# Z-Zheng/ever

Measured on AMD Instinct MI355X. Metric: 512x512 tiles/sec fwd+bwd, FarSeg-R50, higher is better.
Workload: dtype f32; 1 GPU; FarSeg ResNet-50 FPN (FarSegHead defaults, BCE+dice), 3-band 512x512, batch 16/GPU, fwd+bwd+SGD step, inputs resident in HBM; global_batch=16, parallelism=single

## Files before the change

ever_amd/_C.py:

```python
import ctypes as C
import os

_LIB_PATH = os.path.join(os.path.dirname(os.path.abspath(__file__)), 'lib', 'libever_hip.so')
_LIB_PATH = os.environ.get('EVK_LIB', _LIB_PATH)

c_void_p, c_int, c_i32, c_i64, c_u32, c_f32, c_size_t = (
    C.c_void_p, C.c_int, C.c_int32, C.c_int64, C.c_uint32, C.c_float, C.c_size_t)


class ConvDesc(C.Structure):
    _fields_ = [(n, c_i32) for n in (
        'N', 'H', 'W', 'Cin', 'Ho', 'Wo', 'Cout', 'kh', 'kw',
        'stride_h', 'stride_w', 'pad_h', 'pad_w', 'dil_h', 'dil_w')]


class SplitJob(C.Structure):
    _fields_ = [('w', c_void_p), ('out', c_void_p), ('kind', c_i32), ('arg', c_i32 * 13)]


P = c_void_p
_DP = C.POINTER(ConvDesc)
_JP = C.POINTER(SplitJob)

SIGNATURES = {
    'evk_last_error': (C.c_char_p, []),
    'evk_abi_version': (c_int, []),
    'evk_build_arch': (C.c_char_p, []),
    'evk_conv2d_fwd': (c_int, [_DP, P, P, P, P, c_u32, P]),
    'evk_conv2d_dgrad': (c_int, [_DP, P, P, P, P, P]),
    'evk_conv2d_pack_dgrad_weight': (c_int, [_DP, P, P, P]),
    'evk_conv2d_split_weight_bytes': (c_size_t, [_DP, c_i32]),
    'evk_conv2d_split_weight': (c_int, [_DP, P, c_i32, P, P]),
    'evk_conv2d_split_job_count': (c_i32, [_DP, c_i32]),
    'evk_conv2d_split_jobs': (c_int, [_DP, P, c_i32, P, _JP, c_i32]),
    'evk_split_job_pairs': (c_i64, [_JP]),
    'evk_conv2d_route': (c_int, [_DP, c_i32, c_i32, c_u32, c_i32, c_i32, c_i32, C.c_char_p, c_size_t, C.POINTER(c_i32)]),
    'evk_conv2d_wgrad_route': (c_int, [_DP, c_i32, c_u32, C.c_char_p, c_size_t, C.POINTER(c_i32)]),
    'evk_conv2d_split_multi': (c_int, [P, P, c_i32, P]),
    'evk_conv2d_fwd_x3': (c_int, [_DP, P, P, P, P, c_u32, P]),
    'evk_conv2d_stats_max_parts': (c_i32, [_DP]),
    'evk_conv2d_fwd_x3_stats': (c_int, [_DP, P, P, P, P, c_u32, P, c_i32, C.POINTER(c_i32), P]),
    'evk_conv2d_fwd_bf16': (c_int, [_DP, P, P, P, P, c_u32, P, c_i32, C.POINTER(c_i32), P]),
    'evk_conv2d_dgrad_bf16': (c_int, [_DP, P, P, P, P, P]),
    'evk_conv2d_wgrad_bf16': (c_int, [_DP, P, P, P, P, P, c_size_t, P]),
    'evk_conv2d_dgrad_x3': (c_int, [_DP, P, P, P, P, P]),
    'evk_absmax_words': (c_size_t, []),
    'evk_absmax_workspace_bytes': (c_size_t, []),
    'evk_absmax': (c_int, [P, c_i64, P, P, P]),
    'evk_absmax_multi': (c_int, [P, P, c_i32, P, P]),
    'evk_conv2d_split_weight_f16x2': (c_int, [_DP, P, c_i32, P, P, P]),
    'evk_conv2d_split_multi_f16x2': (c_int, [P, P, c_i32, P, P]),
    'evk_conv2d_fwd_f16x2': (c_int, [_DP, P, P, P, P, P, P, P, c_u32, P, c_i32, C.POINTER(c_i32), P, P]),
    'evk_conv2d_dgrad_f16x2': (c_int, [_DP, P, P, P, P, P, P, P, P]),
    'evk_conv2d_wgrad_f16x2': (c_int, [_DP, P, P, P, P, P, P, P, c_size_t, P]),
    'evk_pack_f16x2': (c_int, [P, c_i64, P, P, P]),
    'evk_unpack_f16x2': (c_int, [P, c_i64, P, P, P]),
    'evk_pack_planar_f16x2': (c_int, [P, c_i64, P, P, P]),
    'evk_unpack_planar_f16x2': (c_int, [P, c_i64, P, P, P]),
    'evk_conv2d_dgrad_f16x2_ex': (c_int, [_DP, P, P, P, P, P, P, P, c_u32, P]),
    'evk_conv2d_dgrad_f16x2_masked': (c_int, [_DP, P, P, P, P, P, P, P, P, c_u32, P]),
    'evk_conv2d_wgrad_f16x2_ex': (c_int, [_DP, P, P, P, P, P, P, P, c_size_t, c_u32, P]),
    'evk_conv_transpose2d_fwd': (c_int, [_DP, P, P, P, P, P]),
    'evk_conv_transpose2d_fwd_x3': (c_int, [_DP, P, P, P, P, P]),
    'evk_conv_transpose2d_dgrad': (c_int, [_DP, P, P, P, P]),
    'evk_conv_transpose2d_dgrad_x3': (c_int, [_DP, P, P, P, P]),
    'evk_conv_transpose2d_wgrad_workspace_bytes': (c_size_t, [_DP, c_i32]),
    'evk_conv_transpose2d_wgrad': (c_int, [_DP, P, P, P, P, P, c_size_t, P]),
    'evk_conv_transpose2d_wgrad_x3': (c_int, [_DP, P, P, P, P, P, c_size_t, P]),
    'evk_conv2d_fwd_res': (c_int, [_DP, P, P, P, P, P, c_u32, P]),
    'evk_conv2d_fwd_x3_res': (c_int, [_DP, P, P, P, P, P, c_u32, P]),
    'evk_conv2d_wgrad_x3_workspace_bytes': (c_size_t, [_DP]),
    'evk_conv2d_wgrad_x3': (c_int, [_DP, P, P, P, P, P, c_size_t, P]),
    'evk_conv2d_wgrad_workspace_bytes': (c_size_t, [_DP]),
    'evk_conv2d_wgrad': (c_int, [_DP, P, P, P, P, P, c_size_t, P]),
    'evk_stem_s2d': (c_int, [P, P, c_i32, c_i32, c_i32, c_i32, c_i32, P]),
    'evk_stem_s2d_weight': (c_int, [P, P, c_i32, c_i32, P]),
    'evk_stem_s2d_weight_bwd': (c_int, [P, P, c_i32, c_i32, P]),
    'evk_pad_channels': (c_int, [P, P, c_i64, c_i32, c_i32, P]),
    'evk_unpad_channels': (c_int, [P, P, c_i64, c_i32, c_i32, P]),
    'evk_nchw_to_nhwc': (c_int, [P, P, c_i32, c_i32, c_i32, c_i32, c_i32, P]),
    'evk_nhwc_to_nchw': (c_int, [P, P, c_i32, c_i32, c_i32, c_i32, c_i32, P]),
    'evk_bn_workspace_bytes': (c_size_t, [c_i64, c_i32]),
    'evk_bn_plan': (c_int, [c_i64, c_i32, c_i32, C.POINTER(c_i32)]),
    'evk_bn_fwd_train': (c_int, [P, P, P, P, P, P, c_f32, c_f32, P, P, P, c_i64, c_i32, c_u32, P, c_size_t, P, P]),
    'evk_bn_fwd_train_parts': (c_int, [P, P, P, P, P, P, c_f32, c_f32, P, P, P, c_i64, c_i32, c_u32, P, c_i32, P, c_size_t, P, P]),
    'evk_bn_fwd_train_parts_bits': (c_int, [P, P, P, P, P, P, c_f32, c_f32, P, P, P, c_i64, c_i32, c_u32, P, c_i32, P, c_size_t, P, P, P]),
    'evk_relu_bits_bytes': (c_size_t, [c_i64]),
    'evk_relu_bits_apply': (c_int, [P, P, P, c_i64, P]),
    'evk_bn_fwd_eval': (c_int, [P, P, P, P, P, P, c_f32, P, P, P, c_i64, c_i32, c_u32, P, c_size_t, P, P]),
    'evk_bn_relu_pool_fwd_train_parts': (c_int, [P, P, P, P, P, c_f32, c_f32, P, P, P, P, c_i32, c_i32, c_i32, c_i32, P, c_i32,
                                                 P, c_size_t, P, P]),
    'evk_bn_relu_pool_bwd': (c_int, [P, P, P, P, P, P, P, P, P, P, c_i32, c_i32, c_i32, c_i32, c_i32, P, c_size_t, P, P]),
    'evk_bn_bwd': (c_int, [P, P, P, P, P, P, P, P, P, P, P, c_i64, c_i32, c_u32, c_i32, P, c_size_t, P, P]),
    'evk_stream_fork': (c_int, [P, P]),
    'evk_streams_overlap': (c_int, [P, P, c_i32, P]),
    'evk_bn_relu_dot_plan': (c_int, [c_i64, c_i32, c_i32, C.POINTER(c_i32)]),
    'evk_bn_relu_dot_fwd': (c_int, [P, P, P, P, P, c_i64, c_i32, c_i32, P]),
    'evk_bn_relu_dot_workspace_bytes': (c_size_t, [c_i64, c_i32, c_i32]),
    'evk_bn_relu_dot_bwd': (c_int, [P, P, P, P, P, P, P, P, P, P, P, P, c_i64, c_i32, c_i32, c_u32, P, c_size_t, P, P]),
    'evk_bn_finalize_parts': (c_int, [P, c_i32, c_i32, c_i64, P, P, P, P, c_f32, c_f32, P, P, P, P]),
    'evk_relation_bn_fwd': (c_int, [P, P, P, P, P, P, P, c_i32, c_i32, c_i32, P, P]),
    'evk_relation_bn_parts': (c_i32, [c_i32, c_i32]),
    'evk_relation_bn_workspace_bytes': (c_size_t, [c_i32, c_i32, c_i32]),
    'evk_relation_bn_bwd': (c_int, [P, P, P, P, P, P, P, P, P, P, P, P, c_i32, c_i32, c_i32, P, c_size_t, P]),
    'evk_bn_bwd_from_partials': (c_int, [P, P, P, P, P, P, P, c_i32, P, P, P, c_i64, c_i32, c_u32, c_i32, P, c_size_t, P, P]),
    'evk_bn_bwd_bits': (c_int, [P, P, P, P, P, P, P, P, P, P, P, c_i64, c_i32, c_u32, c_i32, P, c_size_t, P, P, P]),
    'evk_bn_fwd_train_parts_dual': (c_int, [P, P, P, P, P, P, c_f32, c_f32, P, P, P, P, c_f32, c_f32, P, P, P, P, P, c_i64, c_i32,
                                            P, c_i32, P, c_i32, P, c_size_t, P, P, P]),
    'evk_bn_bwd_dual': (c_int, [P, P, P, P, P, P, P, P, P, P, P, P, P, P, P, c_i64, c_i32, c_u32, c_u32, P, c_size_t, P, P, P, P]),
    'evk_bn_bwd_dual_fused': (c_int, [c_u32, c_u32]),
    'evk_relu_fwd': (c_int, [P, P, c_i64, P]),
    'evk_relu_bwd': (c_int, [P, P, P, c_i64, P]),
    'evk_add': (c_int, [P, P, P, c_i64, P]),
    'evk_scale': (c_int, [P, c_f32, P, c_i64, P]),
    'evk_group_weight_expand': (c_int, [P, P, c_i32, c_i32, c_i32, c_i32, P]),
    'evk_group_weight_gather': (c_int, [P, P, c_i32, c_i32, c_i32, c_i32, P]),
    'evk_mul_scale': (c_int, [P, P, c_f32, P, c_i64, P]),
    'evk_gelu_fwd': (c_int, [P, P, c_i64, P]),
    'evk_gelu_bwd': (c_int, [P, P, P, c_i64, P]),
    'evk_maxpool3x3s2_fwd': (c_int, [P, P, P, c_i32, c_i32, c_i32, c_i32, P]),
    'evk_maxpool3x3s2_bwd': (c_int, [P, P, P, c_i32, c_i32, c_i32, c_i32, P]),
    'evk_upsample_nearest2x_add_fwd': (c_int, [P, P, P, c_i32, c_i32, c_i32, c_i32, P, P]),
    'evk_upsample_nearest2x_bwd': (c_int, [P, P, c_i32, c_i32, c_i32, c_i32, P]),
    'evk_subsample2_fwd': (c_int, [P, P, c_i32, c_i32, c_i32, c_i32, P]),
    'evk_subsample2_bwd': (c_int, [P, P, c_i32, c_i32, c_i32, c_i32, P]),
    'evk_upsample_bilinear_fwd': (c_int, [P, P, c_i32, c_i32, c_i32, c_i32, c_i32, c_i32, P]),
    'evk_upsample_bilinear_bwd': (c_int, [P, P, c_i32, c_i32, c_i32, c_i32, c_i32, c_i32, P]),
    'evk_upsample_bilinear_plan': (c_int, [c_i32, c_i32, c_i32, c_i32, c_i32, c_i32, c_i32, c_i32, C.POINTER(c_i32)]),
    'evk_upsample_bilinear_slice_fwd': (c_int, [P, P, c_i32, c_i32, c_i32, c_i32, c_i32, c_i32, c_i32, c_i32, P]),
    'evk_upsample_bilinear_slice_bwd': (c_int, [P, P, c_i32, c_i32, c_i32, c_i32, c_i32, c_i32, c_i32, c_i32, P]),
    'evk_hr_fuse_fwd': (c_int, [P, P, P, c_i32, P, P, P, c_i32, c_i32, c_i32, c_i32, P]),
    'evk_hr_fuse_bwd': (c_int, [P, P, P, P, P, P, c_i32, c_i32, c_i32, c_i32, P]),
    'evk_wfuse_fwd': (c_int, [P, P, c_i32, P, c_i32, c_f32, P, c_i32, c_i32, c_i32, c_i32, P]),
    'evk_wfuse_bwd': (c_int, [P, P, P, c_i32, P, c_i32, c_f32, P, P, P, c_i64, c_i32, c_i32, c_i32, c_i32, P]),
    'evk_wfuse_workspace_bytes': (c_size_t, [c_i32, c_i32, c_i32, c_i32, c_i32]),
    'evk_wfuse_plan': (c_int, [c_i32, c_i32, c_i32, c_i32, c_i32, C.POINTER(c_i32)]),
    'evk_d4_apply': (c_int, [P, P, c_i32, c_i32, c_i32, c_i32, c_i32, P]),
    'evk_d4_merge': (c_int, [P, P, c_i32, P, P, c_i32, c_i32, c_i32, c_i32, c_i32, P]),
    'evk_d4_plan': (c_int, [c_i32, c_i32, c_i32, c_i32, c_i32, C.POINTER(c_i32)]),
    'evk_d4_force_kernel': (c_int, [c_i32]),
    'evk_augment_batch': (c_int, [P, P, c_i32, c_i32, c_i32, c_i32, c_i32, c_i32, P, P, c_i32, c_i32, c_i32, c_i32, P, P, P]),
    'evk_augment_plan': (c_int, [c_i32] * 12 + [C.POINTER(c_i32)]),
    'evk_augment_force_kernel': (c_int, [c_i32]),
    'evk_gap_fwd': (c_int, [P, P, c_i32, c_i32, c_i32, P]),
    'evk_gap_bwd': (c_int, [P, P, c_i32, c_i32, c_i32, P]),
    'evk_relation_fwd': (c_int, [P, P, P, P, P, c_i32, c_i32, c_i32, P]),
    'evk_relation_workspace_bytes': (c_size_t, [c_i32, c_i32, c_i32]),
    'evk_relation_bwd': (c_int, [P, P, P, P, P, P, P, P, c_i32, c_i32, c_i32, P, c_size_t, P]),
    'evk_mean4_fwd': (c_int, [P, P, P, P, P, c_i64, P, P]),
    'evk_loss_stats_doubles': (c_i64, [c_i32]),
    'evk_bce_fwd': (c_int, [P, P, c_i64, c_i64, c_f32, P, P, P]),
    'evk_bce_bwd': (c_int, [P, P, c_i64, c_i64, c_f32, P, P, P, c_i32, P]),
    'evk_bce_fwd_ex': (c_int, [P, P, c_i64, c_i64, c_f32, c_f32, c_i32, P, P, P]),
    'evk_bce_bwd_ex': (c_int, [P, P, c_i64, c_i64, c_f32, c_f32, c_i32, P, P, P, c_i32, P]),
    'evk_soft_ce_fwd': (c_int, [P, P, c_i64, c_i32, P, P, P]),
    'evk_soft_ce_bwd': (c_int, [P, P, c_i64, c_i32, P, P, P]),
    'evk_dice_stats': (c_int, [P, P, c_i64, c_i32, c_i64, P, P]),
    'evk_dice_finish': (c_int, [P, c_i32, c_f32, c_i32, P, P]),
    'evk_dice_bwd': (c_int, [P, P, c_i64, c_i32, c_i64, P, c_f32, c_i32, P, P, c_i32, P]),
    'evk_ce_fwd': (c_int, [P, P, c_i64, c_i32, c_i64, c_f32, P, P, P]),
    'evk_ce_bwd': (c_int, [P, P, c_i64, c_i32, c_i64, c_f32, P, P, P, c_i32, P]),
    'evk_opt_blocks_per_tensor': (c_i32, []),
    'evk_sqnorm_multi': (c_int, [P, P, c_i32, P, c_f32, P, P, P]),
    'evk_sgd_multi': (c_int, [P, P, P, P, c_i32, c_f32, c_f32, c_f32, c_f32, c_i32, c_i32, P, P]),
    'evk_sgd_multi_lr': (c_int, [P, P, P, P, c_i32, c_f32, P, c_f32, c_f32, c_f32, c_i32, c_i32, P, P]),
    'evk_adam_multi': (c_int, [P, P, P, P, P, c_i32, c_f32, c_f32, c_f32, c_f32, c_f32, c_i32, c_f32, c_f32, P, P]),
    'evk_prob_stats_doubles': (c_i64, [c_i32]),
    'evk_prob_stats': (c_int, [P, P, c_i64, c_i32, c_i64, P, P]),
    'evk_prob_stats_bwd': (c_int, [P, P, c_i64, c_i32, c_i64, P, P, P, c_i32, P]),
    'evk_focal_fwd': (c_int, [P, P, c_i64, c_f32, c_f32, c_i32, c_i32, P, P, P]),
    'evk_focal_bwd': (c_int, [P, P, c_i64, c_f32, c_f32, c_i32, c_i32, P, P, P]),
    'evk_confusion_matrix': (c_int, [P, P, c_i64, c_i32, P, P]),
    'evk_confusion_from_logits': (c_int, [P, P, c_i64, c_i32, c_i32, P, P]),
    'evk_gn_workspace_bytes': (c_size_t, [c_i32, c_i64, c_i32, c_i32]),
    'evk_gn_plan': (c_int, [c_i64, c_i32, C.POINTER(c_i32)]),
    'evk_gn_fwd': (c_int, [P, P, P, c_f32, P, P, P, c_i32, c_i64, c_i32, c_i32, c_u32, P, c_size_t, P]),
    'evk_gn_bwd': (c_int, [P, P, P, P, P, P, P, P, P, c_i32, c_i64, c_i32, c_i32, c_u32, P, c_size_t, P]),
    'evk_concat_channels': (c_int, [P, P, P, c_i64, c_i32, c_i32, P]),
    'evk_split_channels': (c_int, [P, P, P, c_i64, c_i32, c_i32, P]),
    'evk_channel_scale': (c_int, [P, P, P, c_i32, c_i64, c_i32, P]),
    'evk_bn_local_stats': (c_int, [P, P, c_i64, c_i32, P, c_size_t, P]),
    'evk_bn_apply_stats': (c_int, [P, P, P, P, P, P, P, c_i64, c_i32, c_u32, P, c_size_t, P]),
    'evk_bn_bwd_local_sums': (c_int, [P, P, P, P, P, P, P, P, P, c_i64, c_i32, c_u32, P, c_size_t, P]),
    'evk_bn_bwd_apply_sums': (c_int, [P, P, P, P, P, P, P, P, P, P, c_i64, c_i32, c_u32, P, c_size_t, P]),
    'evk_pack_multi': (c_int, [P, P, P, c_i32, c_f32, P, P]),
    'evk_ce_pixel_fwd': (c_int, [P, P, c_i64, c_i32, c_i64, P, P]),
    'evk_ce_pixel_bwd': (c_int, [P, P, c_i64, c_i32, c_i64, P, P, P]),
    'evk_ohem_state_bytes': (c_i64, []),
    'evk_ohem_fwd': (c_int, [P, c_i64, c_i64, P, P, P]),
    'evk_ohem_bwd': (c_int, [P, c_i64, P, P, P, P]),
    'evk_depthwise_fwd': (c_int, [_DP, P, P, P, P, c_u32, P]),
    'evk_depthwise_bwd_workspace_bytes': (c_size_t, [_DP]),
    'evk_depthwise_bwd': (c_int, [_DP, P, P, P, P, P, P, P, P, c_size_t, P]),
    'evk_broadcast_hw': (c_int, [P, P, c_i32, c_i64, c_i32, P]),
    'evk_sum_hw': (c_int, [P, P, c_i32, c_i64, c_i32, P]),
    'evk_ln_plan': (c_int, [c_i64, c_i32, C.POINTER(c_i32)]),
    'evk_ln_bwd_workspace_bytes': (c_size_t, [c_i64, c_i32]),
    'evk_ln_fwd': (c_int, [P, P, P, c_f32, P, P, P, c_i64, c_i32, P]),
    'evk_ln_bwd': (c_int, [P, P, P, P, P, P, P, P, c_i64, c_i32, P, c_size_t, P]),
    'evk_scale_residual_fwd': (c_int, [P, P, P, P, P, c_i32, c_i64, c_i32, P]),
    'evk_scale_residual_bwd_workspace_bytes': (c_size_t, [c_i32, c_i64, c_i32]),
    'evk_scale_residual_bwd': (c_int, [P, P, P, P, P, P, c_i32, c_i64, c_i32, P, c_size_t, P]),
}

_lib = None


class HipExtensionMissing(RuntimeError):
    pass


class HipKernelError(RuntimeError):
    pass


def lib_path():
    return _LIB_PATH


def load():
    global _lib
    if _lib is not None:
        return _lib
    if not os.path.exists(_LIB_PATH):
        raise HipExtensionMissing(
            f'{_LIB_PATH} not found: build it with `python -c "import __graft_entry__ as g; g.build()"` '
            f'or `make -C ever_amd/csrc`. ever_amd has no CPU fallback for its kernels.')
    lib = C.CDLL(_LIB_PATH)
    for name, (res, args) in SIGNATURES.items():
        fn = getattr(lib, name)
        fn.restype = res
        fn.argtypes = args
    _lib = lib
    return lib


def check(rc, what=''):
    if rc != 0:
        msg = load().evk_last_error().decode('utf-8', 'replace')
        raise HipKernelError(f'{what} failed with status {rc}: {msg}')


def call(name, *args):
    rc = getattr(load(), name)(*args)
    if rc != 0:
        check(rc, name)
```

ever_amd/csrc/bn.hip:

```cpp
#include "bn_common.hpp"

namespace evk {

__global__ __launch_bounds__(256) void bn_stats_partial_kernel(const float* __restrict__ x, float* __restrict__ partial,
                                                               int64_t rows, int C, int64_t rows_per_blk, int tpc,
                                                               int rl) {
  __shared__ f32x4 red[2][256];
  const int c4 = C >> 2;
  const int tc = threadIdx.x % tpc, tr = threadIdx.x / tpc;
  const int64_t r0 = (int64_t)blockIdx.x * rows_per_blk;
  const int64_t r1 = min(rows, r0 + rows_per_blk);
  for (int cb = tc; cb < c4; cb += tpc) {
    f32x4 s = {0.f, 0.f, 0.f, 0.f}, q = {0.f, 0.f, 0.f, 0.f};
    const f32x4 pv = *reinterpret_cast<const f32x4*>(x + cb * 4);
    if (tr < rl) {
      int64_t r = r0 + tr;
      const int64_t st = rl;
      for (; r + 3 * st < r1; r += 4 * st) {
        const f32x4 v0 = *reinterpret_cast<const f32x4*>(x + r * C + cb * 4) - pv;
        const f32x4 v1 = *reinterpret_cast<const f32x4*>(x + (r + st) * C + cb * 4) - pv;
        const f32x4 v2 = *reinterpret_cast<const f32x4*>(x + (r + 2 * st) * C + cb * 4) - pv;
        const f32x4 v3 = *reinterpret_cast<const f32x4*>(x + (r + 3 * st) * C + cb * 4) - pv;
        s += (v0 + v1) + (v2 + v3);
        q += (v0 * v0 + v1 * v1) + (v2 * v2 + v3 * v3);
// ... 112 lines not shown
    const float* __restrict__ dy, const float* __restrict__ x, const float* __restrict__ xb, const float* __restrict__ y,
    const float* __restrict__ mean, const float* __restrict__ invstd, const float* __restrict__ mean_b,
    const float* __restrict__ invstd_b, const float* __restrict__ gamma, const float* __restrict__ beta,
    float* __restrict__ d_residual, float* __restrict__ partial, float* __restrict__ partial_b, int64_t rows, int C,
    int64_t rows_per_blk, int tpc, int rl, int relu, float* __restrict__ pmax, float* __restrict__ pmax_b,
    const uint32_t* __restrict__ bits) {
  if constexpr (NM == 2) {
    relu = 3;
    d_residual = nullptr;
  }
  __shared__ f32x4 red[2][256];
  const float* const xs[2] = {x, xb};
  const float* const means[2] = {mean, mean_b};
  const float* const invstds[2] = {invstd, invstd_b};
  float* const partials[2] = {partial, partial_b};
  float* const pmaxs[2] = {pmax, pmax_b};
  const f32x4 zero4 = {0.f, 0.f, 0.f, 0.f};
  const int c4 = C >> 2;
  const int tc = threadIdx.x % tpc, tr = threadIdx.x / tpc;
  const int64_t r0 = (int64_t)bn_blk() * rows_per_blk;
  const int64_t r1 = min(rows, r0 + rows_per_blk);
  for (int cb = tc; cb < c4; cb += tpc) {
    f32x4 mu[NM], is[NM], q[NM], xm[NM];
#pragma unroll
    for (int m = 0; m < NM; ++m) {
      mu[m] = *reinterpret_cast<const f32x4*>(means[m] + cb * 4);
      is[m] = *reinterpret_cast<const f32x4*>(invstds[m] + cb * 4);
      q[m] = xm[m] = zero4;
    }
    f32x4 sc = {1.f, 1.f, 1.f, 1.f}, sh = zero4;
    if (relu == 2) {
      const f32x4 one = {1.f, 1.f, 1.f, 1.f};
      const f32x4 g4 = gamma ? *reinterpret_cast<const f32x4*>(gamma + cb * 4) : one;
      const f32x4 b4 = beta ? *reinterpret_cast<const f32x4*>(beta + cb * 4) : zero4;
      sc = g4 * is[0];
      sh = b4 - mu[0] * sc;
    }
    f32x4 s = zero4, gm = zero4;
    if (tr < rl) {
      auto one = [&](const f32x4 gin, const f32x4* xv, const f32x4 yin, size_t off) {
        f32x4 g = gin;
        if (relu == 3) {
          g = relu_bits_mask(g, bits, off >> 2);
        } else if (relu) {
          const f32x4 yy = (relu == 1) ? yin : xv[0] * sc + sh;
          g = relu_mask(g, yy);
        }
        if (d_residual) *reinterpret_cast<f32x4*>(d_residual + off) = g;
        s += g;
        f32x4 xh[NM];
#pragma unroll
        for (int m = 0; m < NM; ++m) {
          xh[m] = (xv[m] - mu[m]) * is[m];
          q[m] += g * xh[m];
        }
        if constexpr (PK) {
          absmax4(gm, g);
#pragma unroll
          for (int m = 0; m < NM; ++m) absmax4(xm[m], xh[m]);
        }
      };
      int64_t r = r0 + tr;
      const int64_t st = rl;
      for (; r + 3 * st < r1; r += 4 * st) {
        size_t o[4];
        f32x4 g[4], xv[4][NM], yv[4];
#pragma unroll
        for (int k = 0; k < 4; ++k) o[k] = (size_t)(r + k * st) * C + cb * 4;
#pragma unroll
        for (int k = 0; k < 4; ++k) g[k] = bp_ld(dy + o[k]);
#pragma unroll
        for (int m = 0; m < NM; ++m)
#pragma unroll
          for (int k = 0; k < 4; ++k) xv[k][m] = bp_ld(xs[m] + o[k]);
#pragma unroll
        for (int k = 0; k < 4; ++k) yv[k] = zero4;
        if (relu == 1) {
#pragma unroll
          for (int k = 0; k < 4; ++k) yv[k] = bp_ld(y + o[k]);
        }
#pragma unroll
        for (int k = 0; k < 4; ++k) one(g[k], xv[k], yv[k], o[k]);
      }
      for (; r < r1; r += st) {
        const size_t o0 = (size_t)r * C + cb * 4;
        f32x4 xv[NM];
        const f32x4 g0 = bp_ld(dy + o0);
#pragma unroll
        for (int m = 0; m < NM; ++m) xv[m] = bp_ld(xs[m] + o0);
        one(g0, xv, (relu == 1) ? bp_ld(y + o0) : zero4, o0);
      }
    }
#pragma unroll
    for (int m = 0; m < NM; ++m) fold_store_record(red, s, q[m], partials[m], bn_blk(), C, cb, tc, tr, tpc, rl);
    if constexpr (PK) {
#pragma unroll
      for (int m = 0; m < NM; ++m) fold_store_maxima(red, gm, xm[m], pmaxs[m], bn_blk(), C, cb, tc, tr, tpc, rl);
    }
  }
}

template <int FC>
__device__ __forceinline__ void bn_bwd_final_body(const float* __restrict__ partial, int nblk, int C,
                                                  double inv_rows, const float* __restrict__ gamma,
                                                  const float* __restrict__ invstd,
                                                  float* __restrict__ dgamma, float* __restrict__ dbeta,
                                                  float* __restrict__ coef, int train,
                                                  uint32_t* __restrict__ amax,
                                                  const float* __restrict__ pmax) {
  if (!pmax) zero_amax(amax);
  float gmax = 0.f, xmax = 0.f;
  if (pmax) {
    __shared__ float mred[4][FC];
    const int tc = threadIdx.x % FC, tl = threadIdx.x / FC;
    const int cc = bn_fin_group() * FC + tc;
    if (cc < C) {
      const float* pm = pmax + cc;
      const size_t st = (size_t)2 * C;
      int b = tl;
      for (; b + 3 * (256 / FC) < nblk; b += 4 * (256 / FC)) {
        const float g0 = pm[b * st], g1 = pm[(b + (256 / FC)) * st], g2 = pm[(b + 2 * (256 / FC)) * st],
                    g3 = pm[(b + 3 * (256 / FC)) * st];
        const float x0 = pm[b * st + C], x1 = pm[(b + (256 / FC)) * st + C], x2 = pm[(b + 2 * (256 / FC)) * st + C],
                    x3 = pm[(b + 3 * (256 / FC)) * st + C];
        gmax = fmaxf(gmax, fmaxf(fmaxf(g0, g1), fmaxf(g2, g3)));
        xmax = fmaxf(xmax, fmaxf(fmaxf(x0, x1), fmaxf(x2, x3)));
      }
      for (; b < nblk; b += (256 / FC)) {
        gmax = fmaxf(gmax, pm[b * st]);
        xmax = fmaxf(xmax, pm[b * st + C]);
      }
    }
    auto mx = [](float a, float b) { return fmaxf(a, b); };
    gmax = fold_channel_lanes<FC>(gmax, mred, mx);
    xmax = fold_channel_lanes<FC>(xmax, mred, mx);
  }
  int c;
  double s, q;
  if (!reduce_partials<FC>(partial, nblk, C, c, s, q)) return;
  if (dbeta) dbeta[c] = (float)s;
  if (dgamma) dgamma[c] = (float)q;
  const float g = gamma ? gamma[c] : 1.f;
  const float k0 = g * invstd[c], k1 = train ? (float)(s * inv_rows) : 0.f, k2 = train ? (float)(q * inv_rows) : 0.f;
  coef[c] = k0;
  coef[C + c] = k1;
  coef[2 * C + c] = k2;
  if (pmax) {
    const float bound = fabsf(k0) * (gmax + fabsf(k1) + xmax * fabsf(k2));
    uint32_t bits = __builtin_bit_cast(uint32_t, bound);
    if (bound != bound) bits = 0x7fc00000u;
    if (bits) atomicMax(&amax[0], bits);
  }
}
struct BnBwdFinalSet {
  const float *partial, *gamma, *invstd;
  float *dgamma, *dbeta, *coef;
  int train;
  uint32_t* amax;
  const float* pmax;
};
template <typename Set, int NR>
struct BnFinalSets {
  Set row[NR];
};
template <typename Set, int NR>
__device__ __forceinline__ Set bn_final_row(const BnFinalSets<Set, NR>& sets) {
  if constexpr (NR == 1) return sets.row[0];
  else return blockIdx.y ? sets.row[1] : sets.row[0];
}
template <int NR>
__global__ __launch_bounds__(256) void bn_bwd_final_kernel(BnFinalSets<BnBwdFinalSet, NR> sets, int nblk, int C, double inv_rows) {
  const BnBwdFinalSet s = bn_final_row(sets);
  bn_bwd_final_body<kFinCh>(s.partial, nblk, C, inv_rows, s.gamma, s.invstd, s.dgamma, s.dbeta, s.coef, s.train, s.amax, s.pmax);
}

struct BnDxCoef {
  f32x4 k0, k1, k2, mu, is;
};
__device__ __forceinline__ BnDxCoef bn_dx_coef(const float* __restrict__ coef, const float* __restrict__ mean,
                                               const float* __restrict__ invstd, int C, int c) {
  return {reinterpret_cast<const f32x4*>(coef)[c], reinterpret_cast<const f32x4*>(coef + C)[c],
          reinterpret_cast<const f32x4*>(coef + 2 * C)[c], reinterpret_cast<const f32x4*>(mean)[c],
          reinterpret_cast<const f32x4*>(invstd)[c]};
}
template <bool PK>
__device__ __forceinline__ f32x4 bn_dx_store(const BnDxCoef& k, const f32x4 g, const f32x4 xv, float* __restrict__ dx, size_t i,
                                             float pk_inv) {
  const f32x4 xh = (xv - k.mu) * k.is;
  const f32x4 out = k.k0 * (g - k.k1 - xh * k.k2);
  if constexpr (PK) {
    reinterpret_cast<u32x4*>(dx)[i] = pack_hl4(out, pk_inv);
  } else {
    reinterpret_cast<f32x4*>(dx)[i] = out;
  }
  return out;
}
template <bool PK>
__global__ __launch_bounds__(256) void bn_bwd_apply_kernel(const float* __restrict__ dy, const float* __restrict__ x,
                                                           const float* __restrict__ y, const float* __restrict__ mean,
                                                           const float* __restrict__ invstd,
                                                           const float* __restrict__ coef,
                                                           const float* __restrict__ gamma,
                                                           const float* __restrict__ beta, float* __restrict__ dx,
                                                           size_t n4, int C, int relu, uint32_t* __restrict__ amax,
                                                           const uint32_t* __restrict__ bits = nullptr) {
  const size_t base = (size_t)bn_blk() * 256;
  const size_t i = base + threadIdx.x;
  const bool valid = i < n4;
  f32x4 out = {0.f, 0.f, 0.f, 0.f};
  float pk_inv = 1.f;
  if constexpr (PK) pk_inv = op_scale(amax[0]).inv;
  if (valid) {
    const int c4 = C >> 2;
    const int c = chunk_of(base, c4);
    const f32x4 one4 = {1.f, 1.f, 1.f, 1.f}, z4 = {0.f, 0.f, 0.f, 0.f};
    const BnDxCoef k = bn_dx_coef(coef, mean, invstd, C, c);
    f32x4 g = bn_ld(dy, i);
    const f32x4 xv = bn_ld(x, i);
    if (relu == 3) {
      g = relu_bits_mask(g, bits, i);
    } else if (relu) {
      f32x4 yy;
      if (relu == 1) {
        yy = reinterpret_cast<const f32x4*>(y)[i];
      } else {
        const f32x4 sc = (gamma ? reinterpret_cast<const f32x4*>(gamma)[c] : one4) * k.is;
        const f32x4 sh = (beta ? reinterpret_cast<const f32x4*>(beta)[c] : z4) - k.mu * sc;
        yy = xv * sc + sh;
      }
      g = relu_mask(g, yy);
    }
    out = bn_dx_store<PK>(k, g, xv, dx, i, pk_inv);
  }
  if constexpr (!PK)
    if (amax) block_absmax(out, valid, amax);
}

template <int FC, int FL>
__device__ __forceinline__ void bn_parts_final_body(const float* __restrict__ parts, int nparts, int C,
                                                    double rows, const float* __restrict__ gamma,
                                                    const float* __restrict__ beta,
                                                    float* __restrict__ running_mean,
                                                    float* __restrict__ running_var, float momentum, float eps,
                                                    float* __restrict__ save_mean, float* __restrict__ save_invstd,
                                                    float* __restrict__ scale_shift,
                                                    uint32_t* __restrict__ amax, int pack) {
  if (!pack) zero_amax(amax);
  float E = 0.f;
  __shared__ double red[4][FC];
  const int tc = threadIdx.x % FC, tl = threadIdx.x / FC;
  const int c = bn_fin_group() * FC + tc;
  double N = 0.0, A = 0.0, B = 0.0, piv = 0.0;
  if (c < C) {
    const size_t st = (size_t)3 * C;
    piv = (double)parts[C + c];
    const float* r = parts + c;
    int b = tl;
    for (; b + 3 * FL < nparts; b += 4 * FL) {
      const float* r0 = r + (size_t)b * st;
      const float* r1 = r0 + (size_t)FL * st;
      const float* r2 = r1 + (size_t)FL * st;
      const float* r3 = r2 + (size_t)FL * st;
      const float n0 = r0[0], m0 = r0[C], q0 = r0[2 * C], n1 = r1[0], m1 = r1[C], q1 = r1[2 * C];
      const float n2 = r2[0], m2 = r2[C], q2 = r2[2 * C], n3 = r3[0], m3 = r3[C], q3 = r3[2 * C];
      const double d0 = (double)m0 - piv, d1 = (double)m1 - piv, d2 = (double)m2 - piv, d3 = (double)m3 - piv;
      N += ((double)n0 + (double)n1) + ((double)n2 + (double)n3);
      A += ((double)n0 * d0 + (double)n1 * d1) + ((double)n2 * d2 + (double)n3 * d3);
      B += (((double)q0 + (double)n0 * d0 * d0) + ((double)q1 + (double)n1 * d1 * d1)) +
           (((double)q2 + (double)n2 * d2 * d2) + ((double)q3 + (double)n3 * d3 * d3));
      if (pack) {
        const float e0 = n0 > 0.f ? sqrtf(q0) + fabsf((float)d0) : 0.f, e1 = n1 > 0.f ? sqrtf(q1) + fabsf((float)d1) : 0.f;
        const float e2 = n2 > 0.f ? sqrtf(q2) + fabsf((float)d2) : 0.f, e3 = n3 > 0.f ? sqrtf(q3) + fabsf((float)d3) : 0.f;
        E = fmaxf(E, fmaxf(fmaxf(e0, e1), fmaxf(e2, e3)));
      }
    }
    for (; b < nparts; b += FL) {
      const float* r0 = r + (size_t)b * st;
      const double n0 = (double)r0[0], d0 = (double)r0[C] - piv;
      N += n0;
      A += n0 * d0;
      B += (double)r0[2 * C] + n0 * d0 * d0;
      if (pack && n0 > 0.0) E = fmaxf(E, sqrtf(r0[2 * C]) + fabsf((float)d0));
    }
  }
  __shared__ float ered[4][FC];
  auto add = [](double a, double b) { return a + b; };
  N = fold_channel_lanes<FC>(N, red, add);
  A = fold_channel_lanes<FC>(A, red, add);
  B = fold_channel_lanes<FC>(B, red, add);
  if (pack) E = fold_channel_lanes<FC>(E, ered, [](float a, float b) { return fmaxf(a, b); });
  if (tl != 0 || c >= C) return;
  const double mean = N > 0.0 ? piv + A / N : 0.0;
  double var = N > 0.0 ? (B - A * A / N) / N : 0.0;
  if (var < 0.0) var = 0.0;
  const float invstd = (float)(1.0 / sqrt(var + (double)eps));
  const float meanf = (float)mean;
  save_mean[c] = meanf;
  save_invstd[c] = invstd;
  const double unbias = rows > 1.0 ? rows / (rows - 1.0) : 1.0;
  if (running_mean) running_mean[c] = (1.f - momentum) * running_mean[c] + momentum * meanf;
  if (running_var) running_var[c] = (1.f - momentum) * running_var[c] + momentum * (float)(var * unbias);
  const float g = gamma ? gamma[c] : 1.f, bb = beta ? beta[c] : 0.f;
  const float sc = g * invstd;
  scale_shift[c] = sc;
  scale_shift[C + c] = bb - meanf * sc;
  if (pack) {
    const float bound = fabsf(sc) * (E * 1.001f + fabsf((float)(piv - mean))) + fabsf(bb);
    uint32_t bits = __builtin_bit_cast(uint32_t, bound);
    if (bound != bound) bits = 0x7fc00000u;
    if (bits) atomicMax(&amax[0], bits);
  }
}
struct BnPartsFinalSet {
  const float* parts;
  int nparts;
  const float *gamma, *beta;
  float *running_mean, *running_var;
  float momentum, eps;
  float *save_mean, *save_invstd, *scale_shift;
  uint32_t* amax;
  int pack;
};
template <int FC, int FL, int NR>
__global__ __launch_bounds__(256) void bn_parts_final_kernel(BnFinalSets<BnPartsFinalSet, NR> sets, int C, double rows) {
  const BnPartsFinalSet s = bn_final_row(sets);
  bn_parts_final_body<FC, FL>(s.parts, s.nparts, C, rows, s.gamma, s.beta, s.running_mean, s.running_var, s.momentum, s.eps,
                              s.save_mean, s.save_invstd, s.scale_shift, s.amax, NR == 1 ? s.pack : 0);
}


static int parts_final_lanes(int nparts) { return nparts >= 1024 ? 256 : (nparts >= 512 ? 128 : 32); }

static void launch_parts_final_sets(hipStream_t st, const BnPartsFinalSet& a, const BnPartsFinalSet* b, int C, double rows) {
  pick<256, 128, 32>(parts_final_lanes(a.nparts), [&](auto FL) {
    constexpr int fl = decltype(FL)::value, fc = 256 / fl;
    const dim3 grid((C + fc - 1) / fc, b ? 2 : 1);
    if (b) hipLaunchKernelGGL((bn_parts_final_kernel<fc, fl, 2>), grid, dim3(256), 0, st, BnFinalSets<BnPartsFinalSet, 2>{{a, *b}}, C, rows);
    else hipLaunchKernelGGL((bn_parts_final_kernel<fc, fl, 1>), grid, dim3(256), 0, st, BnFinalSets<BnPartsFinalSet, 1>{{a}}, C, rows);
    return 0;
  });
}
void launch_parts_final(hipStream_t st, const float* parts, int nparts, int C, double rows, const float* gamma,
                        const float* beta, float* running_mean, float* running_var, float momentum, float eps,
                        float* save_mean, float* save_invstd, float* scale_shift, uint32_t* amax, int pack) {
  const BnPartsFinalSet s = {parts, nparts, gamma, beta, running_mean, running_var, momentum, eps, save_mean, save_invstd,
                             scale_shift, amax, pack};
  launch_parts_final_sets(st, s, nullptr, C, rows);
}

static void launch_bn_bwd_final_sets(hipStream_t st, const BnBwdFinalSet& a, const BnBwdFinalSet* b, int nblk, int C,
                                     int64_t rows) {
  const dim3 grid((C + kFinCh - 1) / kFinCh, b ? 2 : 1);
  const double inv_rows = 1.0 / (double)rows;
  if (b) hipLaunchKernelGGL(bn_bwd_final_kernel<2>, grid, dim3(256), 0, st, BnFinalSets<BnBwdFinalSet, 2>{{a, *b}}, nblk, C, inv_rows);
  else hipLaunchKernelGGL(bn_bwd_final_kernel<1>, grid, dim3(256), 0, st, BnFinalSets<BnBwdFinalSet, 1>{{a}}, nblk, C, inv_rows);
}
void launch_bn_bwd_final(hipStream_t st, const float* partial, int nblk, int C, int64_t rows, const float* gamma,
                         const float* invstd, float* dgamma, float* dbeta, float* coef, int train, uint32_t* amax,
                         const float* pmax) {
  const BnBwdFinalSet s = {partial, gamma, invstd, dgamma, dbeta, coef, train ? 1 : 0, amax, pmax};
  launch_bn_bwd_final_sets(st, s, nullptr, nblk, C, rows);
}

static void launch_bn_apply(hipStream_t st, bool pack, const float* x, const float* residual, const float* scale_shift,
                            float* y, int64_t rows, int C, uint32_t flags, uint32_t* amax, uint32_t* relu_bits = nullptr,
                            const float* scale_shift_b = nullptr) {
  const size_t n4 = (size_t)rows * C / 4;
  const int relu = (flags & EVK_BN_RELU) ? 1 : 0;
  auto launch = [&](auto kernel) {
    hipLaunchKernelGGL(kernel, dim3(oneshot_grid(n4)), dim3(256), 0, st, x, residual, scale_shift, scale_shift_b, y, n4, C, relu,
                       amax, relu_bits);
  };
  if (scale_shift_b) launch(bn_apply_kernel<false, true>);
  else if (pack) launch(bn_apply_kernel<true, false>);
  else launch(bn_apply_kernel<false, false>);
}

static void launch_bn_bwd_partial(hipStream_t st, const BnPlan& pl, const float* dy, const float* x, const float* y,
                                  const float* mean, const float* invstd, const float* gamma, const float* beta,
                                  float* d_residual, float* partial, int64_t rows, int C, int relu, float* pmax,
                                  const uint32_t* bits, const float* xb = nullptr, const float* mean_b = nullptr,
                                  const float* invstd_b = nullptr, float* partial_b = nullptr, float* pmax_b = nullptr) {
  auto launch = [&](auto kernel) {
    hipLaunchKernelGGL(kernel, dim3(pl.nblk), dim3(256), 0, st, dy, x, xb, y, mean, invstd, mean_b, invstd_b, gamma, beta,
                       d_residual, partial, partial_b, rows, C, pl.rows_per_blk, pl.tpc, pl.rl, relu, pmax, pmax_b, bits);
  };
  if (xb) pmax ? launch(bn_bwd_partial_kernel<2, true>) : launch(bn_bwd_partial_kernel<2, false>);
  else pmax ? launch(bn_bwd_partial_kernel<1, true>) : launch(bn_bwd_partial_kernel<1, false>);
}


template <bool PKA, bool PKB>
__global__ __launch_bounds__(256) void bn_bwd_apply_dual_kernel(
    const float* __restrict__ dy, const float* __restrict__ xa, const float* __restrict__ xb,
    const float* __restrict__ mean_a, const float* __restrict__ invstd_a, const float* __restrict__ coef_a,
    const float* __restrict__ mean_b, const float* __restrict__ invstd_b, const float* __restrict__ coef_b,
    float* __restrict__ dxa, float* __restrict__ dxb, size_t n4, int C, uint32_t* __restrict__ amax_a,
    uint32_t* __restrict__ amax_b, const uint32_t* __restrict__ bits) {
  const size_t base = (size_t)bn_blk() * 256;
  const size_t i = base + threadIdx.x;
  const bool valid = i < n4;
  f32x4 outa = {0.f, 0.f, 0.f, 0.f}, outb = {0.f, 0.f, 0.f, 0.f};
  float pk_inv_a = 1.f, pk_inv_b = 1.f;
  if constexpr (PKA) pk_inv_a = op_scale(amax_a[0]).inv;
  if constexpr (PKB) pk_inv_b = op_scale(amax_b[0]).inv;
  if (valid) {
    const int c4 = C >> 2;
    const int c = chunk_of(base, c4);
    const f32x4 g = relu_bits_mask(bn_ld(dy, i), bits, i);
    const BnDxCoef ka = bn_dx_coef(coef_a, mean_a, invstd_a, C, c);
    outa = bn_dx_store<PKA>(ka, g, bn_ld(xa, i), dxa, i, pk_inv_a);
    const BnDxCoef kb = bn_dx_coef(coef_b, mean_b, invstd_b, C, c);
    outb = bn_dx_store<PKB>(kb, g, bn_ld(xb, i), dxb, i, pk_inv_b);
  }
  if constexpr (!PKA)
    if (amax_a) block_absmax(outa, valid, amax_a);
  if constexpr (!PKA && !PKB) __syncthreads();
  if constexpr (!PKB)
    if (amax_b) block_absmax(outb, valid, amax_b);
}

static bool bn_dual_fused(bool pack_a, bool pack_b) { return !(pack_a && !pack_b); }

}

using namespace evk;

extern "C" size_t evk_bn_workspace_bytes(int64_t rows, int32_t C) {
  return rows > 0 && C > 0 ? BnWorkspace::bytes(C) : 0;
}

extern "C" int evk_bn_plan(int64_t rows, int32_t C, int32_t kind, int32_t* out) {
  EVK_REQUIRE(out, EVK_E_INVALID, "bn_plan: null pointer");
  int rc = bn_check("bn_plan", rows, C, nullptr, 0, 0);
  if (rc) return rc;
  EVK_REQUIRE(kind >= 0 && kind <= 2 && (kind == 0 || rows < 0x7fffffffLL), EVK_E_UNSUPPORTED,
              "bn_plan: rows=%lld C=%d kind=%d", (long long)rows, C, kind);
  if (kind == 2) {
    const int fl = parts_final_lanes((int)rows), fc = 256 / fl;
    out[0] = (C + fc - 1) / fc;
    out[2] = fc;
    out[3] = fl;
    out[1] = out[4] = out[5] = 0;
    return EVK_OK;
  }
  const BnPlan pl = kind ? bn_plan(rows, C, 65536, kMaxStatBlocks) : bn_plan(rows, C);
  EVK_REQUIRE(pl.rows_per_blk <= 0x7fffffffLL, EVK_E_UNSUPPORTED, "bn_plan: rows=%lld do not fit the answer", (long long)rows);
  out[0] = pl.nblk;
  out[1] = (int32_t)pl.rows_per_blk;
  out[2] = pl.tpc;
  out[3] = pl.rl;
  out[4] = out[5] = 0;
  if (kind == 1 && rows % 4 == 0) {
    int nblk, qpb;
    bn_quad_split(rows, pl, nblk, qpb);
    out[4] = nblk;
    out[5] = qpb;
  }
  return EVK_OK;
}

extern "C" int evk_bn_fwd_train(const float* x, const float* residual, const float* gamma, const float* beta,
                                float* running_mean, float* running_var, float momentum, float eps, float* y,
                                float* save_mean, float* save_invstd, int64_t rows, int32_t C, uint32_t flags,
                                void* workspace, size_t workspace_bytes, uint32_t* y_absmax, void* stream) {
  EVK_REQUIRE(x && y && save_mean && save_invstd, EVK_E_INVALID, "bn_fwd_train: null pointer");
  int rc = bn_check("bn_fwd_train", rows, C, workspace, workspace_bytes, BnWorkspace::bytes(C));
  if (rc) return rc;
  hipStream_t st = (hipStream_t)stream;
  const BnPlan pl = bn_plan(rows, C);
  const BnWorkspace ws(workspace, C);
  hipLaunchKernelGGL(bn_stats_partial_kernel, dim3(pl.nblk), dim3(256), 0, st, x, ws.partial, rows, C, pl.rows_per_blk,
                     pl.tpc, pl.rl);
  rc = check_launch("bn_stats_partial");
  if (rc) return rc;
  const double unbias = rows > 1 ? (double)rows / (double)(rows - 1) : 1.0;
  hipLaunchKernelGGL(bn_stats_final_kernel, dim3((C + kFinCh - 1) / kFinCh), dim3(256), 0, st, x, ws.partial, pl.nblk, C,
                     1.0 / (double)rows, unbias, gamma, beta, running_mean, running_var, momentum, eps, save_mean,
                     save_invstd, ws.coef, y_absmax);
  rc = check_launch("bn_stats_final");
  if (rc) return rc;
  launch_bn_apply(st, false, x, residual, ws.coef, y, rows, C, flags, y_absmax);
  return check_launch("bn_apply");
}

extern "C" int evk_bn_fwd_train_parts_bits(const float* x, const float* residual, const float* gamma, const float* beta,
                                           float* running_mean, float* running_var, float momentum, float eps, float* y,
                                           float* save_mean, float* save_invstd, int64_t rows, int32_t C, uint32_t flags,
                                           const float* parts, int32_t nparts, void* workspace, size_t workspace_bytes,
                                           uint32_t* y_absmax, uint32_t* relu_bits, void* stream) {
  EVK_REQUIRE(x && y && save_mean && save_invstd && parts && nparts > 0, EVK_E_INVALID, "bn_fwd_train_parts: bad argument");
  int rc = bn_check("bn_fwd_train_parts", rows, C, workspace, workspace_bytes, BnWorkspace::bytes(C));
  if (rc) return rc;
  const bool pack = (flags & EVK_BN_PACK_Y) != 0;
  EVK_REQUIRE(!pack || (y_absmax && !residual), EVK_E_INVALID,
              "bn_fwd_train_parts: EVK_BN_PACK_Y needs y_absmax (slots zero on entry) and no residual");
  hipStream_t st = (hipStream_t)stream;
  float* scale_shift = BnWorkspace(workspace, C).coef;
  launch_parts_final(st, parts, nparts, C, (double)rows, gamma, beta, running_mean, running_var, momentum, eps, save_mean,
                     save_invstd, scale_shift, y_absmax, pack ? 1 : 0);
  rc = check_launch("bn_parts_final");
  if (rc) return rc;
  launch_bn_apply(st, pack, x, residual, scale_shift, y, rows, C, flags, y_absmax, relu_bits);
  return check_launch("bn_apply");
// ... 314 lines not shown
```

ever_amd/csrc/bn_common.hpp:

```cpp
#pragma once
#include "x3_common.hpp"

namespace evk {

__device__ __forceinline__ unsigned bn_blk() { return gridDim.x - 1u - blockIdx.x; }

__device__ __forceinline__ int bn_fin_group() { return xcd_remap((int)blockIdx.x, (int)gridDim.x); }

__device__ __forceinline__ f32x4 bn_ld(const float* p, size_t i) {
  return __builtin_nontemporal_load(reinterpret_cast<const f32x4*>(p) + i);
}

constexpr int kMaxStatBlocks = 2048;

__device__ __forceinline__ void zero_amax(uint32_t* __restrict__ amax) {
  if (amax && blockIdx.x == 0 && threadIdx.x < kAmaxSlots) amax[threadIdx.x * kAmaxStride] = 0;
}

struct BnPlan {
  int nblk;
  int64_t rows_per_blk;
  int tpc, rl;
};
inline BnPlan bn_plan(int64_t rows, int C, int64_t per_override = 0, int64_t cap_override = 0) {
// ... 2 lines not shown
  p.tpc = c4 < 256 ? c4 : 256;
  p.rl = 256 / p.tpc;
  constexpr int64_t per = 32768;
  const int64_t per_e = per_override > 0 ? per_override : per;
  int64_t nb = (rows * (int64_t)C + per_e - 1) / per_e;
  constexpr int64_t cap = 512;
  if (nb > (cap_override > 0 ? cap_override : cap)) nb = cap_override > 0 ? cap_override : cap;
  if (nb > kMaxStatBlocks) nb = kMaxStatBlocks;
  if (nb < 1) nb = 1;
  int64_t rpb = (rows + nb - 1) / nb;
  rpb = ((rpb + p.rl - 1) / p.rl) * p.rl;
  p.rows_per_blk = rpb;
  p.nblk = (int)((rows + rpb - 1) / rpb);
  return p;
}

inline void bn_quad_split(int64_t rows, const BnPlan& pl, int& nblk, int& qpb) {
  const int quads = (int)(rows / 4);
  qpb = (quads + pl.nblk - 1) / pl.nblk;
  qpb = ((qpb + pl.rl - 1) / pl.rl) * pl.rl;
  nblk = (quads + qpb - 1) / qpb;
}

inline unsigned oneshot_grid(size_t n4) { return (unsigned)((n4 + 255) / 256); }

struct BnWorkspace {
  float *partial, *coef, *pmax;
  static size_t bytes(int C) { return ((size_t)kMaxStatBlocks * 4 * C + 8 * (size_t)C) * sizeof(float); }
  BnWorkspace(void* ws, int C)
      : partial((float*)ws), coef(partial + (size_t)kMaxStatBlocks * 2 * C), pmax(coef + 8 * (size_t)C) {}
};

inline int bn_check(const char* what, int64_t rows, int32_t C, const void* ws, size_t ws_bytes, size_t need) {
  EVK_REQUIRE(rows > 0 && C > 0 && C % 4 == 0 && C <= 2048, EVK_E_UNSUPPORTED, "%s: rows=%lld C=%d", what, (long long)rows,
              C);
  EVK_REQUIRE(!need || (ws && ws_bytes >= need), EVK_E_WORKSPACE, "%s: workspace too small", what);
  return EVK_OK;
}

#define EVK_BN_LAUNCH_PK(kernel, pack, grid, lds, st, ...)                                   \
  do {                                                                                       \
    if (pack) hipLaunchKernelGGL((kernel<true>), grid, dim3(256), lds, st, __VA_ARGS__);     \
    else hipLaunchKernelGGL((kernel<false>), grid, dim3(256), lds, st, __VA_ARGS__);         \
  } while (0)

__device__ __forceinline__ f32x4 relu_mask(f32x4 g, const f32x4 yy) {
  g.x = yy.x > 0.f ? g.x : 0.f; g.y = yy.y > 0.f ? g.y : 0.f;
  g.z = yy.z > 0.f ? g.z : 0.f; g.w = yy.w > 0.f ? g.w : 0.f;
  return g;
}

__device__ __forceinline__ void fold_store_record(f32x4 (*red)[256], f32x4 s, f32x4 q, float* rec, size_t blk, int C, int cb,
                                                  int tc, int tr, int tpc, int rl) {
  red[0][threadIdx.x] = s;
  red[1][threadIdx.x] = q;
  __syncthreads();
  if (tr == 0) {
    for (int k = 1; k < rl; ++k) {
      s += red[0][k * tpc + tc];
      q += red[1][k * tpc + tc];
    }
    float* o = rec + blk * 2 * C;
    *reinterpret_cast<f32x4*>(o + cb * 4) = s;
    *reinterpret_cast<f32x4*>(o + C + cb * 4) = q;
  }
  __syncthreads();
}

__device__ __forceinline__ void max4(f32x4& m, const f32x4 v) {
  m.x = fmaxf(m.x, v.x); m.y = fmaxf(m.y, v.y); m.z = fmaxf(m.z, v.z); m.w = fmaxf(m.w, v.w);
}
__device__ __forceinline__ void absmax4(f32x4& m, const f32x4 v) {
  m.x = fmaxf(m.x, fabsf(v.x)); m.y = fmaxf(m.y, fabsf(v.y)); m.z = fmaxf(m.z, fabsf(v.z)); m.w = fmaxf(m.w, fabsf(v.w));
}

__device__ __forceinline__ void fold_store_maxima(f32x4 (*red)[256], f32x4 gm, f32x4 xm, float* rec, size_t blk, int C, int cb,
                                                  int tc, int tr, int tpc, int rl) {
  red[0][threadIdx.x] = gm;
  red[1][threadIdx.x] = xm;
  __syncthreads();
  if (tr == 0) {
    for (int k = 1; k < rl; ++k) {
      max4(gm, red[0][k * tpc + tc]);
      max4(xm, red[1][k * tpc + tc]);
    }
    float* o = rec + blk * 2 * C;
    *reinterpret_cast<f32x4*>(o + cb * 4) = gm;
    *reinterpret_cast<f32x4*>(o + C + cb * 4) = xm;
  }
  __syncthreads();
}

constexpr int kFinCh = 8;
template <int FC, typename T, typename Op>
__device__ __forceinline__ T fold_channel_lanes(T v, T (*lds)[FC], Op op) {
#pragma unroll
  for (int o = FC; o < 64; o <<= 1) v = op(v, __shfl_xor(v, o, 64));
  const int lane = threadIdx.x & 63, w = threadIdx.x >> 6;
  if (lane < FC) lds[w][lane] = v;
  __syncthreads();
  const int tc = threadIdx.x % FC;
  const T r = op(op(lds[0][tc], lds[1][tc]), op(lds[2][tc], lds[3][tc]));
  __syncthreads();
  return r;
}
template <int FC = kFinCh>
__device__ __forceinline__ bool reduce_partials(const float* __restrict__ partial, int nblk, int C, int& c, double& s,
                                                double& q) {
  __shared__ double red[4][FC];
  const int tc = threadIdx.x % FC, tl = threadIdx.x / FC;
  c = bn_fin_group() * FC + tc;
  s = 0.0;
  q = 0.0;
  if (c < C) {
    const float* ps = partial + c;
    const size_t st = (size_t)2 * C;
    int b = tl;
    for (; b + 3 * (256 / FC) < nblk; b += 4 * (256 / FC)) {
      const float s0 = ps[b * st], s1 = ps[(b + (256 / FC)) * st], s2 = ps[(b + 2 * (256 / FC)) * st],
                  s3 = ps[(b + 3 * (256 / FC)) * st];
      const float q0 = ps[b * st + C], q1 = ps[(b + (256 / FC)) * st + C], q2 = ps[(b + 2 * (256 / FC)) * st + C],
                  q3 = ps[(b + 3 * (256 / FC)) * st + C];
      s += ((double)s0 + (double)s1) + ((double)s2 + (double)s3);
      q += ((double)q0 + (double)q1) + ((double)q2 + (double)q3);
    }
    for (; b < nblk; b += (256 / FC)) {
      s += (double)ps[b * st];
      q += (double)ps[b * st + C];
    }
  }
  auto add = [](double a, double b) { return a + b; };
  s = fold_channel_lanes<FC>(s, red, add);
  q = fold_channel_lanes<FC>(q, red, add);
  return tl == 0 && c < C;
}

__device__ __forceinline__ void block_absmax(const f32x4 v, bool valid, uint32_t* __restrict__ amax) {
  __shared__ uint32_t red[4];
  uint32_t m = 0;
  if (valid) {
    m = __builtin_bit_cast(uint32_t, fmaxf(fmaxf(fabsf(v.x), fabsf(v.y)), fmaxf(fabsf(v.z), fabsf(v.w))));
    if (v.x != v.x || v.y != v.y || v.z != v.z || v.w != v.w) m = 0x7fc00000u;
  }
#pragma unroll
  for (int o = 32; o > 0; o >>= 1) m = max(m, (uint32_t)__shfl_xor((int)m, o, 64));
  if ((threadIdx.x & 63) == 0) red[threadIdx.x >> 6] = m;
  __syncthreads();
  if (threadIdx.x == 0) {
    const uint32_t t = max(max(red[0], red[1]), max(red[2], red[3]));
    if (t) atomicMax(&amax[(blockIdx.x & (kAmaxSlots - 1)) * kAmaxStride], t);
  }
}

void launch_parts_final(hipStream_t st, const float* parts, int nparts, int C, double rows, const float* gamma,
                        const float* beta, float* running_mean, float* running_var, float momentum, float eps,
                        float* save_mean, float* save_invstd, float* scale_shift, uint32_t* amax, int pack);
void launch_bn_bwd_final(hipStream_t st, const float* partial, int nblk, int C, int64_t rows, const float* gamma,
                         const float* invstd, float* dgamma, float* dbeta, float* coef, int train, uint32_t* amax,
                         const float* pmax);

}
```

ever_amd/csrc/conv_wgrad.hip:

```cpp
#include "wgrad_common.hpp"
#include <stdlib.h>

namespace evk {

#ifndef EVK_SK_NT
#define EVK_SK_NT 1
#endif
#if EVK_SK_NT
#define SK_LD(p) __builtin_nontemporal_load(p)
#else
#define SK_LD(p) (*(p))
#endif
__global__ __launch_bounds__(256) void splitk_reduce_kernel(const float* __restrict__ ws, float* __restrict__ out, size_t n4,
                                                            int splitk, size_t stride4, int lanes) {
  __shared__ f32x4 red[256];
  const f32x4* w4 = reinterpret_cast<const f32x4*>(ws);
  f32x4* o4 = reinterpret_cast<f32x4*>(out);
  const int epb = 256 / lanes;
  const int e = threadIdx.x % epb, l = threadIdx.x / epb;
  for (size_t i0 = (size_t)blockIdx.x * epb; i0 < n4; i0 += (size_t)gridDim.x * epb) {
    const size_t i = i0 + e;
    f32x4 s = {0.f, 0.f, 0.f, 0.f};
    if (i < n4) {
      int z = l;
      for (; z + 3 * lanes < splitk; z += 4 * lanes) {
        const f32x4 a = SK_LD(w4 + (size_t)z * stride4 + i), b = SK_LD(w4 + (size_t)(z + lanes) * stride4 + i);
        const f32x4 c = SK_LD(w4 + (size_t)(z + 2 * lanes) * stride4 + i), d = SK_LD(w4 + (size_t)(z + 3 * lanes) * stride4 + i);
        s += (a + b) + (c + d);
      }
      for (; z < splitk; z += lanes) s += SK_LD(w4 + (size_t)z * stride4 + i);
    }
    if (lanes > 1) {
      red[threadIdx.x] = s;
      __syncthreads();
      if (l == 0 && i < n4) {
        for (int k = 1; k < lanes; ++k) s += red[k * epb + e];
        o4[i] = s;
      }
      __syncthreads();
    } else if (i < n4) {
      o4[i] = s;
    }
  }
}

__global__ __launch_bounds__(256) void colsum_partial_kernel(const float* __restrict__ src, float* __restrict__ partial,
                                                             int64_t rows, int C, int64_t rows_per_blk) {
  __shared__ f32x4 red[256];
  const int c4 = C >> 2;
  const int tpc = min(c4, 256);
  const int rl = 256 / tpc;
  const int tc = threadIdx.x % tpc, tr = threadIdx.x / tpc;
  const int64_t r0 = (int64_t)blockIdx.x * rows_per_blk;
  const int64_t r1 = min(rows, r0 + rows_per_blk);
  for (int cb = tc; cb < c4; cb += tpc) {
    f32x4 s = {0.f, 0.f, 0.f, 0.f};
    if (tr < rl)
      for (int64_t r = r0 + tr; r < r1; r += rl) s += *reinterpret_cast<const f32x4*>(src + r * C + cb * 4);
    red[threadIdx.x] = s;
    __syncthreads();
    if (tr == 0) {
      for (int k = 1; k < rl; ++k) s += red[k * tpc + tc];
      *reinterpret_cast<f32x4*>(partial + (size_t)blockIdx.x * C + cb * 4) = s;
    }
    __syncthreads();
  }
}
__global__ __launch_bounds__(256) void colsum_final_kernel(const float* __restrict__ partial, float* __restrict__ out,
                                                           int nblk, int C) {
  __shared__ double red[32][8];
  const int tc = threadIdx.x & 7, tl = threadIdx.x >> 3;
  const int c = xcd_remap((int)blockIdx.x, (int)gridDim.x) * 8 + tc;
  double s = 0.0;
  if (c < C) {
    int b = tl;
    for (; b + 96 < nblk; b += 128) {
      const float a0 = partial[(size_t)b * C + c], a1 = partial[(size_t)(b + 32) * C + c];
      const float a2 = partial[(size_t)(b + 64) * C + c], a3 = partial[(size_t)(b + 96) * C + c];
      s += ((double)a0 + (double)a1) + ((double)a2 + (double)a3);
    }
    for (; b < nblk; b += 32) s += (double)partial[(size_t)b * C + c];
  }
  red[tl][tc] = s;
  __syncthreads();
  if (tl == 0 && c < C) {
    for (int k = 1; k < 32; ++k) s += red[k][tc];
    out[c] = (float)s;
  }
}

WGradPlan plan_wgrad(const evk_conv_desc* d, int x3, int planes, int tr, int shared) {
  WGradPlan pl;
  const int Ktot = d->kh * d->kw * d->Cin;
  const int M = d->N * d->Ho * d->Wo;
  pl.bm = d->Cout <= 64 ? 64 : 128;
  pl.bn = Ktot <= 64 ? 64 : 128;
  static const bool tune = getenv("EVK_TUNE") != nullptr;
  auto knob = [&](const char* name, int dflt, int lo) {
    const char* v = tune ? getenv(name) : nullptr;
    const int k = (v && *v) ? atoi(v) : dflt;
    return k < lo ? lo : k;
  };
  const int ws_mode = knob("EVK_WG_WS", 1, 0);
  const bool fits32 = (long long)d->N * d->H * d->W * d->Cin * 4 < 0x7fffffffLL &&
                      (long long)d->N * d->Ho * d->Wo * d->Cout * 4 < 0x7fffffffLL;
  const int ws_min = knob("EVK_WG_WS_MINCOUT", 128, 1);
  pl.ws = (x3 && ws_mode && d->Cout >= ws_min && Ktot >= 256 && fits32) ? 1 : 0;
  if (tr) { pl.ws = 1; pl.bm = 128; }
  if (pl.ws) pl.bn = 256;
  if (tr == 2) pl.bn = 9 * 64;
  pl.tiles_co = ceil_div(d->Cout, pl.bm);
  pl.tiles_k = tr == 2 ? d->Cin / 64 : ceil_div(Ktot, pl.bn);
  const int tiles = pl.tiles_co * pl.tiles_k;
  const int rounds = knob("EVK_WG_ROUNDS", 1, 1), min_chunk = knob("EVK_WG_MINCHUNK", 256, 32);
  const int lds_kb = 2 * BKP * (pl.bm + pl.bn) * 4 / 1024;
  const int per_cu = pl.ws ? 1 : x3 ? (pl.bm + pl.bn >= 256 ? 3 : 4)
                        : (lds_kb >= 64 ? 2 : (lds_kb >= 48 ? 3 : 4));
  const int fill = (shared && pl.ws) ? knob("EVK_WG_SHARED_FILL", 50, 1) : 100;
  const int slots = 256 * per_cu * (fill > 0 && fill <= 100 ? fill : 100) / 100;
  int maxsplit = ceil_div(M, min_chunk);
  int sk = (rounds * slots) / tiles;
  if (sk > maxsplit) sk = maxsplit;
  if (sk < 1) sk = 1;
  int chunk = ceil_div(M, sk);
  chunk = ((chunk + BKP - 1) / BKP) * BKP;
  pl.chunk = chunk;
  pl.splitk = ceil_div(M, chunk);
  return pl;
}
static int colsum_blocks(int64_t rows) {
  int64_t b = (rows + 255) / 256;
  return (int)(b > 1024 ? 1024 : (b < 1 ? 1 : b));
}

size_t colsum_workspace_bytes(int64_t rows, int c) { return (size_t)colsum_blocks(rows) * c * sizeof(float) + 256; }
int launch_colsum(const float* src, float* out, int64_t rows, int c, float* workspace, hipStream_t st) {
  const int nblk = colsum_blocks(rows);
  const int64_t rpb = (rows + nblk - 1) / nblk;
  hipLaunchKernelGGL(colsum_partial_kernel, dim3(nblk), dim3(256), 0, st, src, workspace, rows, c, rpb);
  int rc = check_launch("colsum_partial");
  if (rc) return rc;
  hipLaunchKernelGGL(colsum_final_kernel, dim3((c + 7) / 8), dim3(256), 0, st, (const float*)workspace, out, nblk, c);
  return check_launch("colsum_final");
}

}

using namespace evk;

static size_t wgrad_ws_bytes(const evk_conv_desc* d, int x3) {
  if (!d) return 0;
  const WGradPlan pl = plan_wgrad(d, x3), pl2 = plan_wgrad(d, x3, 2);
  const size_t Ktot = (size_t)d->kh * d->kw * d->Cin;
  int sk = pl.splitk > pl2.splitk ? pl.splitk : pl2.splitk;
  if (x3 && d->Cin % 64 == 0) {
    for (int tr = 1; tr <= 2; ++tr) { const int sk3 = plan_wgrad(d, x3, 2, tr).splitk; sk = sk > sk3 ? sk : sk3; }
  }
  size_t a = sk > 1 ? (size_t)sk * d->Cout * Ktot * sizeof(float) : 0;
  size_t b = (size_t)colsum_blocks((int64_t)d->N * d->Ho * d->Wo) * d->Cout * sizeof(float);
  return (a > b ? a : b) + 256;
}

extern "C" size_t evk_conv2d_wgrad_workspace_bytes(const evk_conv_desc* d) { return wgrad_ws_bytes(d, 0); }
extern "C" size_t evk_conv2d_wgrad_x3_workspace_bytes(const evk_conv_desc* d) { return wgrad_ws_bytes(d, 1); }

namespace evk {

int route_wgrad(const evk_conv_desc* d, int planes, uint32_t flags, WGradRoute* r) {
  EVK_REQUIRE(d && r, EVK_E_INVALID, "conv2d_wgrad: null pointer");
  EVK_REQUIRE(planes >= 0 && planes <= 3, EVK_E_INVALID, "conv2d_wgrad: arithmetic %d (0 fp32, 1 bf16, 2 f16x2, 3 bf16x3)", planes);
  EVK_REQUIRE(d->Cin % 4 == 0 && d->Cout % 4 == 0, EVK_E_UNSUPPORTED,
              "conv2d_wgrad: Cin=%d and Cout=%d must be multiples of 4", d->Cin, d->Cout);
  EVK_REQUIRE((long long)d->N * d->H * d->W * d->Cin < 0x7fffffffLL &&
                  (long long)d->N * d->Ho * d->Wo * d->Cout < 0x7fffffffLL,
              EVK_E_UNSUPPORTED, "conv2d_wgrad: tensors of 2^31 or more elements are not supported");
  EVK_REQUIRE(planes == 2 || flags == 0, EVK_E_INVALID, "conv2d_wgrad: flags 0x%x belong to the f16x2 arithmetic", flags);
  const int planar = (flags & (EVK_CONV_X_PLANAR | EVK_CONV_DY_PLANAR)) ? 1 : 0;
  EVK_REQUIRE(!planar || ((flags & EVK_CONV_X_PLANAR) && (flags & EVK_CONV_DY_PLANAR) && planes == 2),
              EVK_E_UNSUPPORTED, "conv2d_wgrad: planar operands come in pairs (x and dy), f16x2 only, no bias gradient");
  EVK_REQUIRE(!planar || wgrad_tr_applicable(d, planes), EVK_E_UNSUPPORTED,
              "conv2d_wgrad: planar operands need Cin %% 64 == 0, Cout %% 64 == 0 and Wo %% 8 == 0 "
              "(Cin=%d Cout=%d Wo=%d) and tensors below 2 GiB", d->Cin, d->Cout, d->Wo);
  const int x3 = planes != 0;
  const int nine = planar && wgrad_tr_nine_tap(d) ? 1 : 0;
  WGradRoute o{};
  o.plan = plan_wgrad(d, x3, x3 ? planes : 3, planar ? 1 + nine : 0, (flags & EVK_CONV_WGRAD_SHARED) ? 1 : 0);
  o.kernel = planar ? WGradKernel::Tr : !x3 ? WGradKernel::Fp32 : o.plan.ws ? WGradKernel::X3Ws : WGradKernel::X3;
  o.pkx = (flags & EVK_CONV_X_PACKED) ? 1 : 0;
  o.pkd = (flags & EVK_CONV_DY_PACKED) ? 1 : 0;
  o.w8 = d->Wo % 8 == 0;
  o.nt = nine ? 9 : 1;
  o.npx = planes == 2 && (o.pkx || o.pkd) && o.kernel == WGradKernel::X3 ? 4 : planes;
  *r = o;
  return EVK_OK;
}

void wgrad_kernel_name(const WGradRoute& r, char* buf, size_t n) {
  auto tf = [](int v) { return v ? "true" : "false"; };
  switch (r.kernel) {
    case WGradKernel::Fp32: snprintf(buf, n, "conv_wgrad_kernel<%d, %d, 2, 2>", r.plan.bm, r.plan.bn); break;
    case WGradKernel::X3: snprintf(buf, n, "conv_wgrad_x3_kernel<%d, %d, 2, 2, %d>", r.plan.bm, r.plan.bn, r.npx); break;
    case WGradKernel::X3Ws:
      snprintf(buf, n, "conv_wgrad_x3ws_kernel<%d, %d, %d, %s, %s, %s>", r.plan.bm, r.plan.bn, r.npx, tf(r.w8), tf(r.pkx), tf(r.pkd));
      break;
    case WGradKernel::Tr: snprintf(buf, n, "conv_wgrad_tr_kernel<%d>", r.nt); break;
  }
}

}

static int conv_wgrad_any(const evk_conv_desc* d, const float* x, const float* dy, float* dw, float* dbias,
                          void* workspace, size_t workspace_bytes, void* stream, int x3, int planes = 3,
                          const uint32_t* x_scale = nullptr, const uint32_t* dy_scale = nullptr, uint32_t pk_flags = 0) {
  EVK_REQUIRE(d && x && dy && dw, EVK_E_INVALID, "conv2d_wgrad: null pointer");
  WGradRoute route;
  int rc = route_wgrad(d, x3 ? planes : 0, pk_flags, &route);
  if (rc) return rc;
  const WGradPlan& pl = route.plan;
  EVK_REQUIRE(workspace_bytes >= wgrad_ws_bytes(d, x3) && (workspace || workspace_bytes == 0), EVK_E_WORKSPACE,
              "conv2d_wgrad: workspace %zu < %zu", workspace_bytes, wgrad_ws_bytes(d, x3));
  hipStream_t st = (hipStream_t)stream;
  const int planar = route.kernel == WGradKernel::Tr ? 1 : 0;
  EVK_REQUIRE(!(planar && dbias), EVK_E_UNSUPPORTED, "conv2d_wgrad: planar operands come in pairs (x and dy), f16x2 only, no bias gradient");
  WGradArgs a{};
  a.planes = planes;
  a.planar = planar;
  a.x_scale = x_scale; a.dy_scale = dy_scale;
  a.x_packed = route.pkx;
  a.dy_packed = route.pkd;
  EVK_REQUIRE(!(a.dy_packed && dbias), EVK_E_UNSUPPORTED, "conv2d_wgrad: the bias gradient needs dy as fp32");
  a.x = x; a.dy = dy;
  a.N = d->N; a.H = d->H; a.W = d->W; a.Cin = d->Cin; a.Ho = d->Ho; a.Wo = d->Wo; a.Cout = d->Cout;
  a.kh = d->kh; a.kw = d->kw; a.cpt = d->Cin / 4;
  a.sh = d->stride_h; a.sw = d->stride_w; a.ph = d->pad_h; a.pw = d->pad_w; a.dh = d->dil_h; a.dw = d->dil_w;
  a.M = d->N * d->Ho * d->Wo;
  a.Ktot = d->kh * d->kw * d->Cin;
  a.chunk = pl.chunk; a.tiles_co = pl.tiles_co; a.tiles_k = pl.tiles_k; a.splitk = pl.splitk;
  a.fd_hw = make_fastdiv((uint32_t)(d->Ho * d->Wo));
  a.fd_w = make_fastdiv((uint32_t)d->Wo);
  a.out = pl.splitk > 1 ? (float*)workspace : dw;
  switch (route.kernel) {
    case WGradKernel::Tr: rc = launch_wgrad_tr(a, route, st); break;
    case WGradKernel::X3:
    case WGradKernel::X3Ws: rc = launch_wgrad_x3(a, route, st); break;
    default: rc = launch_wgrad_f32(a, route, st);
  }
  if (rc) return rc;
  if (pl.splitk > 1) {
    const size_t n = (size_t)d->Cout * a.Ktot;
    const size_t n4 = n / 4;
    int lanes = 1;
    while (lanes < 64 && lanes * 2 <= pl.splitk && n4 * (size_t)lanes < 131072) lanes *= 2;
    const size_t epb = 256 / lanes;
    const int blocks = (int)((n4 + epb - 1) / epb > 4096 ? 4096 : (n4 + epb - 1) / epb);
    hipLaunchKernelGGL(splitk_reduce_kernel, dim3(blocks), dim3(256), 0, st, (const float*)workspace, dw, n4,
                       pl.splitk, n4, lanes);
    rc = check_launch("splitk_reduce");
    if (rc) return rc;
  }
  if (dbias) rc = launch_colsum(dy, dbias, a.M, d->Cout, (float*)workspace, st);
  return rc;
}

extern "C" int evk_conv2d_wgrad(const evk_conv_desc* d, const float* x, const float* dy, float* dw, float* dbias,
                                void* workspace, size_t workspace_bytes, void* stream) {
  return conv_wgrad_any(d, x, dy, dw, dbias, workspace, workspace_bytes, stream, 0);
}

extern "C" int evk_conv2d_wgrad_bf16(const evk_conv_desc* d, const float* x, const float* dy, float* dw, float* dbias,
                                     void* workspace, size_t workspace_bytes, void* stream) {
  EVK_REQUIRE(d && d->Cin % 4 == 0 && d->Cout % 4 == 0, EVK_E_UNSUPPORTED, "conv2d_wgrad_bf16: channels must be multiples of 4");
  return conv_wgrad_any(d, x, dy, dw, dbias, workspace, workspace_bytes, stream, 1, 1);
}

extern "C" int evk_conv2d_wgrad_f16x2(const evk_conv_desc* d, const float* x, const uint32_t* x_absmax, const float* dy,
                                      const uint32_t* dy_absmax, float* dw, float* dbias, void* workspace,
                                      size_t workspace_bytes, void* stream) {
  EVK_REQUIRE(d && d->Cin % 4 == 0 && d->Cout % 4 == 0, EVK_E_UNSUPPORTED, "conv2d_wgrad_f16x2: channels must be multiples of 4");
  EVK_REQUIRE(x_absmax && dy_absmax, EVK_E_INVALID, "conv2d_wgrad_f16x2: null scales");
  return conv_wgrad_any(d, x, dy, dw, dbias, workspace, workspace_bytes, stream, 1, 2, x_absmax, dy_absmax);
}

extern "C" int evk_conv2d_wgrad_f16x2_ex(const evk_conv_desc* d, const void* x, const uint32_t* x_absmax, const void* dy,
                                         const uint32_t* dy_absmax, float* dw, float* dbias, void* workspace,
                                         size_t workspace_bytes, uint32_t flags, void* stream) {
  EVK_REQUIRE(d && d->Cin % 4 == 0 && d->Cout % 4 == 0, EVK_E_UNSUPPORTED, "conv2d_wgrad_f16x2_ex: channels must be multiples of 4");
  EVK_REQUIRE(x_absmax && dy_absmax, EVK_E_INVALID, "conv2d_wgrad_f16x2_ex: null scales");
  EVK_REQUIRE((flags & ~kWGradFlags) == 0, EVK_E_INVALID,
              "conv2d_wgrad_f16x2_ex: unknown flag 0x%x", flags);
  return conv_wgrad_any(d, reinterpret_cast<const float*>(x), reinterpret_cast<const float*>(dy), dw, dbias, workspace,
                        workspace_bytes, stream, 1, 2, x_absmax, dy_absmax, flags);
}

extern "C" int evk_conv2d_wgrad_x3(const evk_conv_desc* d, const float* x, const float* dy, float* dw, float* dbias,
                                   void* workspace, size_t workspace_bytes, void* stream) {
// ... 24 lines not shown
```

ever_amd/csrc/relation.hip:

```cpp
#include "stream_common.hpp"

namespace evk {

__device__ __forceinline__ f32x4 bn_relu4(const f32x4 z, const f32x4 sc, const f32x4 sh) {
  f32x4 y = z * sc + sh;
  y.x = fmaxf(y.x, 0.f); y.y = fmaxf(y.y, 0.f); y.z = fmaxf(y.z, 0.f); y.w = fmaxf(y.w, 0.f);
  return y;
}
template <bool BN>
__device__ __forceinline__ f32x4 relation_act(const float* __restrict__ z, const float* __restrict__ ss, int C, int cb) {
  const f32x4 v = *reinterpret_cast<const f32x4*>(z + cb * 4);
  if (!BN) return v;
  return bn_relu4(v, *reinterpret_cast<const f32x4*>(ss + cb * 4), *reinterpret_cast<const f32x4*>(ss + C + cb * 4));
}
template <bool BN>
__global__ __launch_bounds__(256) void relation_fwd_kernel(const float* __restrict__ scene, const float* __restrict__ zc,
                                                           const float* __restrict__ ssc, const float* __restrict__ zf,
                                                           const float* __restrict__ ssf, float* __restrict__ out,
                                                           float* __restrict__ r, int N, int HW, int C,
                                                           uint32_t* __restrict__ amax) {
  const int c4 = C >> 2;
  const int lane = threadIdx.x & 63;
  const size_t npix = (size_t)N * HW;
  const size_t wstride = (size_t)gridDim.x * 4;
  uint32_t m = 0;
  for (size_t pix = (size_t)blockIdx.x * 4 + (threadIdx.x >> 6); pix < npix; pix += wstride) {
    const size_t n = pix / HW;
    const float* sc = scene + n * C;
    const float* ct = zc + pix * C;
    float dot = 0.f;
    for (int cb = lane; cb < c4; cb += 64) {
      const f32x4 a = *reinterpret_cast<const f32x4*>(sc + cb * 4);
      const f32x4 b = relation_act<BN>(ct, ssc, C, cb);
      dot += a.x * b.x + a.y * b.y + a.z * b.z + a.w * b.w;
    }
    dot = wave_sum(dot);
    const float rv = 1.f / (1.f + expf(-dot));
    if (lane == 0) r[pix] = rv;
    const float* ft = zf + pix * C;
    float* o = out + pix * C;
    for (int cb = lane; cb < c4; cb += 64) {
      const f32x4 v = relation_act<BN>(ft, ssf, C, cb) * rv;
      *reinterpret_cast<f32x4*>(o + cb * 4) = v;
      if (BN) m = abs4_bits(m, v);
    }
  }
  if (BN && amax) commit_absmax(amax, m);
}

__global__ __launch_bounds__(256) void relation_bwd_kernel(const float* __restrict__ dout,
                                                           const float* __restrict__ scene,
                                                           const float* __restrict__ content,
                                                           const float* __restrict__ feat, const float* __restrict__ r,
                                                           float* __restrict__ dcontent, float* __restrict__ dfeat,
                                                           float* __restrict__ partial, int HW, int C, int pix_per_blk,
                                                           int nblk) {
  extern __shared__ __attribute__((aligned(16))) float sacc[];
  const int c4 = C >> 2;
  const int lane = threadIdx.x & 63, wave = threadIdx.x >> 6;
  const int n = blockIdx.y;
  const int p0 = blockIdx.x * pix_per_blk, p1 = min(HW, p0 + pix_per_blk);
  const float* sc = scene + (size_t)n * C;
  float* myacc = sacc + wave * C;
  for (int c = lane; c < C; c += 64) myacc[c] = 0.f;
  for (int p = p0 + wave; p < p1; p += 4) {
    const size_t pix = (size_t)n * HW + p;
    const float rv = r[pix];
    const float* d_o = dout + pix * C;
    const float* ft = feat + pix * C;
    const float* ct = content + pix * C;
    float dot = 0.f;
    for (int cb = lane; cb < c4; cb += 64) {
      const f32x4 a = *reinterpret_cast<const f32x4*>(d_o + cb * 4);
      const f32x4 b = *reinterpret_cast<const f32x4*>(ft + cb * 4);
      dot += a.x * b.x + a.y * b.y + a.z * b.z + a.w * b.w;
      *reinterpret_cast<f32x4*>(dfeat + pix * C + cb * 4) = a * rv;
    }
    dot = wave_sum(dot);
    const float dz = dot * rv * (1.f - rv);
    for (int cb = lane; cb < c4; cb += 64) {
      const f32x4 s4 = *reinterpret_cast<const f32x4*>(sc + cb * 4);
      const f32x4 c4v = *reinterpret_cast<const f32x4*>(ct + cb * 4);
      *reinterpret_cast<f32x4*>(dcontent + pix * C + cb * 4) = s4 * dz;
      f32x4* a = reinterpret_cast<f32x4*>(myacc + cb * 4);
      *a = *a + c4v * dz;
    }
  }
  __syncthreads();
  float* o = partial + ((size_t)n * nblk + blockIdx.x) * C;
  for (int c = threadIdx.x; c < C; c += 256) o[c] = (sacc[c] + sacc[C + c]) + (sacc[2 * C + c] + sacc[3 * C + c]);
}
__global__ __launch_bounds__(256) void relation_dscene_final_kernel(const float* __restrict__ partial,
                                                                    float* __restrict__ dscene, int nblk, int C) {
  __shared__ double red[32][8];
  const int tc = threadIdx.x & 7, tl = threadIdx.x >> 3;
  const int c = blockIdx.x * 8 + tc;
  const int n = blockIdx.y;
  double s = 0.0;
  if (c < C)
    for (int b = tl; b < nblk; b += 32) s += (double)partial[((size_t)n * nblk + b) * C + c];
  red[tl][tc] = s;
  __syncthreads();
  if (tl == 0 && c < C) {
    for (int k = 1; k < 32; ++k) s += red[k][tc];
    dscene[(size_t)n * C + c] = (float)s;
  }
}

template <int NCH>
__global__ __launch_bounds__(256) void relation_bn_bwd_kernel(
    const float* __restrict__ dout, const float* __restrict__ scene, const float* __restrict__ zc,
    const float* __restrict__ ssc, const float* __restrict__ mic, const float* __restrict__ zf, const float* __restrict__ ssf,
    const float* __restrict__ mif, const float* __restrict__ r, float* __restrict__ gc, float* __restrict__ gf,
    float* __restrict__ partial, float* __restrict__ bnp_c, float* __restrict__ bnm_c, float* __restrict__ bnp_f,
    float* __restrict__ bnm_f, int HW, int C, int pix_per_blk, int nblk) {
  extern __shared__ __attribute__((aligned(16))) float sacc[];
  const int c4 = C >> 2;
  const int lane = threadIdx.x & 63, wave = threadIdx.x >> 6;
  const int n = blockIdx.y;
  const int p0 = blockIdx.x * pix_per_blk, p1 = min(HW, p0 + pix_per_blk);
  const float* sc = scene + (size_t)n * C;
  const f32x4 zero4 = {0.f, 0.f, 0.f, 0.f};
  f32x4 acc[NCH][9];
  f32x4 s4[NCH], scc[NCH], shc[NCH], muc[NCH], isc[NCH], scf[NCH], shf[NCH], muf[NCH], isf[NCH];
#pragma unroll
  for (int j = 0; j < NCH; ++j) {
    const int cb = lane + 64 * j;
    const bool ok = cb < c4;
#pragma unroll
    for (int k = 0; k < 9; ++k) acc[j][k] = zero4;
    s4[j] = ok ? *reinterpret_cast<const f32x4*>(sc + cb * 4) : zero4;
    scc[j] = ok ? *reinterpret_cast<const f32x4*>(ssc + cb * 4) : zero4;
    shc[j] = ok ? *reinterpret_cast<const f32x4*>(ssc + C + cb * 4) : zero4;
    muc[j] = ok ? *reinterpret_cast<const f32x4*>(mic + cb * 4) : zero4;
    isc[j] = ok ? *reinterpret_cast<const f32x4*>(mic + C + cb * 4) : zero4;
    scf[j] = ok ? *reinterpret_cast<const f32x4*>(ssf + cb * 4) : zero4;
    shf[j] = ok ? *reinterpret_cast<const f32x4*>(ssf + C + cb * 4) : zero4;
    muf[j] = ok ? *reinterpret_cast<const f32x4*>(mif + cb * 4) : zero4;
    isf[j] = ok ? *reinterpret_cast<const f32x4*>(mif + C + cb * 4) : zero4;
  }
  auto amax4 = [](f32x4& m, const f32x4 v) {
    m.x = fmaxf(m.x, fabsf(v.x)); m.y = fmaxf(m.y, fabsf(v.y)); m.z = fmaxf(m.z, fabsf(v.z)); m.w = fmaxf(m.w, fabsf(v.w));
  };
  for (int p = p0 + wave; p < p1; p += 4) {
    const size_t pix = (size_t)n * HW + p;
    const float rv = r[pix];
    f32x4 a[NCH], zfv[NCH], zcv[NCH];
#pragma unroll
    for (int j = 0; j < NCH; ++j) {
      const int cb = lane + 64 * j;
      const bool ok = cb < c4;
      a[j] = ok ? *reinterpret_cast<const f32x4*>(dout + pix * C + cb * 4) : zero4;
      zfv[j] = ok ? *reinterpret_cast<const f32x4*>(zf + pix * C + cb * 4) : zero4;
      zcv[j] = ok ? *reinterpret_cast<const f32x4*>(zc + pix * C + cb * 4) : zero4;
    }
    float dot = 0.f;
#pragma unroll
    for (int j = 0; j < NCH; ++j) {
      const int cb = lane + 64 * j;
      const f32x4 y = bn_relu4(zfv[j], scf[j], shf[j]);
      dot += a[j].x * y.x + a[j].y * y.y + a[j].z * y.z + a[j].w * y.w;
      f32x4 g = a[j] * rv;
      g.x = y.x > 0.f ? g.x : 0.f; g.y = y.y > 0.f ? g.y : 0.f; g.z = y.z > 0.f ? g.z : 0.f; g.w = y.w > 0.f ? g.w : 0.f;
      if (cb < c4) *reinterpret_cast<f32x4*>(gf + pix * C + cb * 4) = g;
      const f32x4 xh = (zfv[j] - muf[j]) * isf[j];
      acc[j][5] += g;
      acc[j][6] += g * xh;
      amax4(acc[j][7], g);
      amax4(acc[j][8], xh);
    }
    dot = wave_sum(dot);
    const float dz = dot * rv * (1.f - rv);
#pragma unroll
    for (int j = 0; j < NCH; ++j) {
      const int cb = lane + 64 * j;
      const f32x4 y = bn_relu4(zcv[j], scc[j], shc[j]);
      f32x4 g = s4[j] * dz;
      g.x = y.x > 0.f ? g.x : 0.f; g.y = y.y > 0.f ? g.y : 0.f; g.z = y.z > 0.f ? g.z : 0.f; g.w = y.w > 0.f ? g.w : 0.f;
      if (cb < c4) *reinterpret_cast<f32x4*>(gc + pix * C + cb * 4) = g;
      acc[j][0] += y * dz;
      const f32x4 xh = (zcv[j] - muc[j]) * isc[j];
      acc[j][1] += g;
      acc[j][2] += g * xh;
      amax4(acc[j][3], g);
      amax4(acc[j][4], xh);
    }
  }
  float* my = sacc + (size_t)wave * 9 * C;
#pragma unroll
  for (int j = 0; j < NCH; ++j) {
    const int cb = lane + 64 * j;
    if (cb < c4)
#pragma unroll
      for (int k = 0; k < 9; ++k) *reinterpret_cast<f32x4*>(my + (size_t)k * C + cb * 4) = acc[j][k];
  }
  __syncthreads();
  const size_t blk = (size_t)n * nblk + blockIdx.x;
  const size_t W9 = (size_t)9 * C;
  for (int c = threadIdx.x; c < C; c += 256) {
    auto fold = [&](int k) { return (sacc[k * C + c] + sacc[W9 + k * C + c]) + (sacc[2 * W9 + k * C + c] + sacc[3 * W9 + k * C + c]); };
    auto fmx = [&](int k) {
      return fmaxf(fmaxf(sacc[k * C + c], sacc[W9 + k * C + c]), fmaxf(sacc[2 * W9 + k * C + c], sacc[3 * W9 + k * C + c]));
    };
    partial[blk * C + c] = fold(0);
    bnp_c[blk * 2 * C + c] = fold(1);
    bnp_c[blk * 2 * C + C + c] = fold(2);
    bnm_c[blk * 2 * C + c] = fmx(3);
    bnm_c[blk * 2 * C + C + c] = fmx(4);
    bnp_f[blk * 2 * C + c] = fold(5);
    bnp_f[blk * 2 * C + C + c] = fold(6);
    bnm_f[blk * 2 * C + c] = fmx(7);
    bnm_f[blk * 2 * C + C + c] = fmx(8);
  }
}

static int relation_blocks(int HW) {
  constexpr int ppb = 64, cap = 256;
  int b = (HW + ppb - 1) / ppb;
  return b > cap ? cap : (b < 1 ? 1 : b);
}

template <typename F>
static int relation_bwd_launch(const char* what, const float* partial, float* dscene, int N, int HW, int C, hipStream_t st,
                               F&& launch) {
  const int nblk = relation_blocks(HW);
  const int ppb = (HW + nblk - 1) / nblk;
  launch(nblk, ppb);
  int rc = check_launch(what);
  if (rc) return rc;
  hipLaunchKernelGGL(relation_dscene_final_kernel, dim3((C + 7) / 8, N), dim3(256), 0, st, partial, dscene, nblk, C);
  return check_launch("relation_dscene_final");
}
static size_t relation_records(int N, int HW) { return N > 0 && HW > 0 ? (size_t)N * relation_blocks(HW) : 0; }

}

using namespace evk;

extern "C" int evk_relation_fwd(const float* scene, const float* content, const float* feat, float* out, float* r,
                                int32_t N, int32_t HW, int32_t C, void* stream) {
  EVK_REQUIRE(scene && content && feat && out && r && nhwc4_ok(N, HW, 1, C), EVK_E_INVALID, "relation_fwd: bad argument");
  hipLaunchKernelGGL(relation_fwd_kernel<false>, dim3(grid_for((size_t)N * HW, 4, 8192)), dim3(256), 0, (hipStream_t)stream,
                     scene, content, (const float*)nullptr, feat, (const float*)nullptr, out, r, N, HW, C, (uint32_t*)nullptr);
  return check_launch("relation_fwd");
}
extern "C" int evk_relation_bn_fwd(const float* scene, const float* zc, const float* scale_shift_c, const float* zf,
                                   const float* scale_shift_f, float* out, float* r, int32_t N, int32_t HW, int32_t C,
                                   uint32_t* out_absmax, void* stream) {
  EVK_REQUIRE(scene && zc && scale_shift_c && zf && scale_shift_f && out && r && nhwc4_ok(N, HW, 1, C), EVK_E_INVALID,
              "relation_bn_fwd: bad argument");
  hipLaunchKernelGGL(relation_fwd_kernel<true>, dim3(grid_for((size_t)N * HW, 4, 8192)), dim3(256), 0, (hipStream_t)stream,
                     scene, zc, scale_shift_c, zf, scale_shift_f, out, r, N, HW, C, out_absmax);
  return check_launch("relation_bn_fwd");
}
extern "C" int32_t evk_relation_bn_parts(int32_t N, int32_t HW) { return (int32_t)relation_records(N, HW); }
extern "C" size_t evk_relation_bn_workspace_bytes(int32_t N, int32_t HW, int32_t C) {
  return C > 0 ? relation_records(N, HW) * C * 9 * sizeof(float) : 0;
}
extern "C" int evk_relation_bn_bwd(const float* dout, const float* scene, const float* zc, const float* scale_shift_c,
                                   const float* mean_invstd_c, const float* zf, const float* scale_shift_f,
                                   const float* mean_invstd_f, const float* r, float* dscene, float* gc, float* gf,
                                   int32_t N, int32_t HW, int32_t C, void* workspace, size_t workspace_bytes,
                                   void* stream) {
  EVK_REQUIRE(dout && scene && zc && scale_shift_c && mean_invstd_c && zf && scale_shift_f && mean_invstd_f && r && dscene &&
                  gc && gf,
              EVK_E_INVALID, "relation_bn_bwd: null pointer");
  EVK_REQUIRE(nhwc4_ok(N, HW, 1, C) && C <= 448, EVK_E_UNSUPPORTED, "relation_bn_bwd: C=%d", C);
  EVK_REQUIRE(workspace && workspace_bytes >= evk_relation_bn_workspace_bytes(N, HW, C), EVK_E_WORKSPACE,
              "relation_bn_bwd: workspace too small");
  const size_t nb = relation_records(N, HW);
  float* w = (float*)workspace;
  float* partial = w;
  float* bnp_c = w + nb * C;
  float* bnm_c = w + nb * 3 * C;
  float* bnp_f = w + nb * 5 * C;
  float* bnm_f = w + nb * 7 * C;
  hipStream_t st = (hipStream_t)stream;
  const size_t lds = (size_t)4 * 9 * C * sizeof(float);
  EVK_REQUIRE(lds <= 64 * 1024, EVK_E_UNSUPPORTED, "relation_bn_bwd: C=%d does not fit the LDS", C);
  return relation_bwd_launch("relation_bn_bwd", partial, dscene, N, HW, C, st, [&](int nblk, int ppb) {
    pick<1, 2, 4>((C / 4 + 63) / 64, [&](auto NCH) {
      hipLaunchKernelGGL(relation_bn_bwd_kernel<NCH()>, dim3(nblk, N), dim3(256), lds, st, dout, scene, zc, scale_shift_c,
                         mean_invstd_c, zf, scale_shift_f, mean_invstd_f, r, gc, gf, partial, bnp_c, bnm_c, bnp_f, bnm_f, HW, C,
                         ppb, nblk);
      return 0;
    });
  });
}
extern "C" size_t evk_relation_workspace_bytes(int32_t N, int32_t HW, int32_t C) {
  return C > 0 ? relation_records(N, HW) * C * sizeof(float) : 0;
}
extern "C" int evk_relation_bwd(const float* dout, const float* scene, const float* content, const float* feat,
                                const float* r, float* dscene, float* dcontent, float* dfeat, int32_t N, int32_t HW,
                                int32_t C, void* workspace, size_t workspace_bytes, void* stream) {
  EVK_REQUIRE(dout && scene && content && feat && r && dscene && dcontent && dfeat, EVK_E_INVALID,
              "relation_bwd: null pointer");
  EVK_REQUIRE(nhwc4_ok(N, HW, 1, C) && C <= 4096, EVK_E_UNSUPPORTED, "relation_bwd: C=%d", C);
  EVK_REQUIRE(workspace && workspace_bytes >= evk_relation_workspace_bytes(N, HW, C), EVK_E_WORKSPACE,
              "relation_bwd: workspace too small");
  hipStream_t st = (hipStream_t)stream;
  return relation_bwd_launch("relation_bwd", (const float*)workspace, dscene, N, HW, C, st, [&](int nblk, int ppb) {
    hipLaunchKernelGGL(relation_bwd_kernel, dim3(nblk, N), dim3(256), 4 * C * sizeof(float), st, dout, scene, content, feat, r,
                       dcontent, dfeat, (float*)workspace, HW, C, ppb, nblk);
  });
}
```

ever_amd/csrc/wgrad_common.hpp:

```cpp
#pragma once
#include "common.hpp"

namespace evk {

struct WGradArgs {
  const float* x;
  const float* dy;
  float* out;
  int N, H, W, Cin, Ho, Wo, Cout;
  int kh, kw, cpt;
  int sh, sw, ph, pw, dh, dw;
  int M, Ktot;
  int chunk;
  int tiles_co, tiles_k, splitk;
  FastDiv fd_hw, fd_w;
  int planes;
  const uint32_t* x_scale;
  const uint32_t* dy_scale;
  int x_packed, dy_packed;
  int planar;
  int reserved;
};

constexpr int BKP = 32;

struct WGradPlan {
  int bm, bn, tiles_co, tiles_k, splitk, chunk;
  int ws;
};
WGradPlan plan_wgrad(const evk_conv_desc* d, int x3, int planes = 3, int tr = 0, int shared = 0);

enum class WGradKernel { Fp32, X3, X3Ws, Tr };
struct WGradRoute {
  WGradKernel kernel;
  int npx;
  int w8, pkx, pkd;
  int nt;
  WGradPlan plan;
};
int route_wgrad(const evk_conv_desc* d, int planes, uint32_t flags, WGradRoute* r);
void wgrad_kernel_name(const WGradRoute& r, char* buf, size_t n);
int launch_wgrad_f32(const WGradArgs& a, const WGradRoute& r, hipStream_t stream);
int launch_wgrad_x3(const WGradArgs& a, const WGradRoute& r, hipStream_t stream);
int launch_wgrad_x3ws(const WGradArgs& a, const WGradRoute& r, hipStream_t stream);
bool wgrad_tr_applicable(const evk_conv_desc* d, int planes);
bool wgrad_tr_nine_tap(const evk_conv_desc* d);
int launch_wgrad_tr(const WGradArgs& a, const WGradRoute& r, hipStream_t stream);

constexpr uint32_t kWGradFlags = EVK_CONV_X_PACKED | EVK_CONV_DY_PACKED | EVK_CONV_X_PLANAR | EVK_CONV_DY_PLANAR | EVK_CONV_WGRAD_SHARED;

size_t colsum_workspace_bytes(int64_t rows, int c);
int launch_colsum(const float* src, float* out, int64_t rows, int c, float* workspace, hipStream_t st);

}
```

ever_amd/hip/conv.py:

```python
import ctypes
import os

import torch
from torch.autograd import Function
from torch.autograd.function import once_differentiable

from .. import _C
from . import timing, weight_planes
from .workspace import workspace
from ._base import (
    HipPathError, _BN_EPILOGUE, _PACKED, _amax_zeroed, _entry, _f16x2, _is_packed, _lazy_bits, _note_amax, _planes_math,
    _ptr, _require_cuda, _stream, _weight_planes, absmax_bits, as_nhwc, empty_nhwc, get_conv_math, is_nhwc,
    materialize_lazy, observers_active, relu_bits_stats, _conv_out,
)
from .streams import (
    _WGRAD_BATCH, _WGRAD_EARLY_MODE, _WGRAD_OWNED, _WGRAD_QUEUE, _WGRAD_SHARED, _WGRAD_SHARED_ON, _WGRAD_STREAM,
    _note_param_use, _wgrad_hold, _wgrad_side_stream, flush_wgrad_queue,
)


_WGRAD_PACK_MARGIN = float(os.environ.get('EVK_WGRAD_PACK_MARGIN', '0.0'))
_WGRAD_PACK_GAIN = float(os.environ.get('EVK_WGRAD_PACK_GAIN', '1.0'))


# ... 8 lines not shown
    return gain * t_kernel - t_pack > _WGRAD_PACK_MARGIN * t_kernel


_WGRAD_TR = os.environ.get('EVK_WGRAD_TR', '1') != '0'
_WGRAD_TR_MIN_HW = int(os.environ.get('EVK_WGRAD_TR_MIN_HW', str(128 * 128)))


def _wgrad_planar_pays(d, need_db=False):
    return (_WGRAD_TR and _f16x2() and not need_db and d.kh == 3 and d.kw == 3 and d.stride_h == 1 and d.stride_w == 1
            and d.pad_h == 1 and d.pad_w == 1 and d.dil_h == 1 and d.dil_w == 1 and d.W % 32 == 0 and d.Cin % 64 == 0
            and d.Cout % 64 == 0 and d.Cout >= 128 and d.H * d.W >= _WGRAD_TR_MIN_HW
            and d.N * d.H * d.W * max(d.Cin, d.Cout) * 4 < 2 ** 31)


def _pair(v):
    return (v, v) if isinstance(v, int) else tuple(v)


def _conv_desc(n, h, w, cin, cout, kh, kw, stride, padding, dilation):
    sh, sw = stride
    ph, pw = padding
    dh, dw = dilation
    return _C.ConvDesc(n, h, w, cin, _conv_out(h, kh, sh, ph, dh), _conv_out(w, kw, sw, pw, dw), cout, kh, kw, sh, sw, ph, pw,
                       dh, dw)


def _pad4(c):
    return (c + 3) // 4 * 4


def conv_channel_padding(cin, cout, planes):
    cin_p = _pad4(cin)
    narrow8 = bool(planes and cin_p == cin and cout % 8 != 0 and cout < 8 and os.environ.get('EVK_NARROW_X3', '1') != '0')
    return cin_p, (8 if narrow8 else _pad4(cout)), narrow8


def _pad_last(t2d_ptr, rows, c, cp, device):
    out = torch.empty((rows, cp), device=device, dtype=torch.float32)
    _C.call('evk_pad_channels', t2d_ptr, out.data_ptr(), rows, c, cp, _stream())
    return out


def _weight_ohwi(weight):
    if is_nhwc(weight):
        return weight
    o, i, kh, kw = weight.shape
    wc = weight.contiguous()
    out = empty_nhwc(o, i, kh, kw, weight.device)
    _C.call('evk_nchw_to_nhwc', wc.data_ptr(), out.data_ptr(), o, i, kh, kw, i, _stream())
    return out


class _ConvState:
    __slots__ = ('desc', 'relu', 'cin', 'has_bias', 'flops', 'abytes', 'w_stride', 'xk', 'w_ohwi', 'y', 'weight',
                 'w_alias', 'scope', 'bn_parts', 'bias_leaf')


def _stash(states):
    out = []
    for cs in states:
        cs.w_alias = cs.w_ohwi is None or cs.w_ohwi.data_ptr() == cs.weight.data_ptr()
        out += [cs.xk, cs.y, cs.weight, None if cs.w_alias else cs.w_ohwi]
        cs.xk = cs.y = cs.weight = cs.w_ohwi = None
    return out


def _unstash(states, saved):
    for i, cs in enumerate(states):
        cs.xk, cs.y, cs.weight, w = saved[4 * i:4 * i + 4]
        cs.w_ohwi = cs.weight.detach() if cs.w_alias else w


def _drop(states):
    for cs in states:
        cs.xk = cs.y = cs.weight = cs.w_ohwi = cs.bias_leaf = None


def _stats_request(d, dev):
    cap = int(_C.load().evk_conv2d_stats_max_parts(ctypes.byref(d)))
    return torch.empty((cap * 3 * d.Cout,), device=dev, dtype=torch.float32), cap


def _launch_forward(d, x_ptr, xbits, pl_ptr, wabs_ptr, bias, y, flags, st, parts=None, cap=0, ybits=None, x_pk=False):
    nparts = ctypes.c_int32(0)
    if wabs_ptr is not None:
        _C.call('evk_conv2d_fwd_f16x2', ctypes.byref(d), x_ptr, xbits.data_ptr(), pl_ptr, wabs_ptr, _ptr(bias), None,
                y.data_ptr(), flags | (2 if x_pk else 0), _ptr(parts), cap, ctypes.byref(nparts), _ptr(ybits), st)
    elif get_conv_math() == 'bf16':
        _C.call('evk_conv2d_fwd_bf16', ctypes.byref(d), x_ptr, pl_ptr, _ptr(bias), y.data_ptr(), flags, _ptr(parts), cap,
                ctypes.byref(nparts), st)
    elif parts is not None:
        _C.call('evk_conv2d_fwd_x3_stats', ctypes.byref(d), x_ptr, pl_ptr, _ptr(bias), y.data_ptr(), flags, parts.data_ptr(), cap,
                ctypes.byref(nparts), st)
    else:
        _C.call('evk_conv2d_fwd_x3', ctypes.byref(d), x_ptr, pl_ptr, _ptr(bias), y.data_ptr(), flags, st)
    return int(nparts.value)


def _conv_forward(x, weight, bias, stride, padding, dilation, relu, want_stats=False):
    n, cin, h, w = x.shape
    cout, cin_w, kh, kw = weight.shape
    if cin_w != cin:
        raise ValueError(f'conv2d: input has {cin} channels but weight expects {cin_w} (groups != 1 unsupported)')
    dev, st = x.device, _stream()
    w_ohwi = _weight_ohwi(weight.detach())
    cin_p = _pad4(cin)
    xk, wk = x, w_ohwi
    if cin_p != cin:
        xk = _pad_last(x.data_ptr(), n * h * w, cin, cin_p, dev)
        wk = _pad_last(w_ohwi.data_ptr(), cout * kh * kw, cin, cin_p, dev)
    x_ptr, w_ptr = xk.data_ptr(), wk.data_ptr()
    d = _conv_desc(n, h, w, cin_p, cout, kh, kw, stride, padding, dilation)
    x_pk = _is_packed(x)
    if x_pk and not (_f16x2() and cin_p == cin and cin % 8 == 0 and n * d.Ho * d.Wo > 32):
        raise HipPathError('conv2d: a packed activation reached a convolution that cannot read it '
                           f'(math {get_conv_math()}, Cin {cin}, {n * d.Ho * d.Wo} output rows)')
    y = empty_nhwc(n, cout, d.Ho, d.Wo, dev)
    cs = _ConvState()
    cs.scope = timing.current_scope()
    cs.flops = 2.0 * n * d.Ho * d.Wo * cout * cin * kh * kw
    cs.abytes = 4.0 * (n * h * w * cin + n * d.Ho * d.Wo * cout + cout * cin * kh * kw)
    small_m = n * d.Ho * d.Wo <= 32
    bn_parts = None
    if _planes_math() and cin_p == cin and cin % 8 == 0 and not small_m:
        pl_ptr, wabs_ptr, _keep = _weight_planes(weight, w_ohwi, w_ptr, d, 0, st, dev)
        xbits = absmax_bits(x, st) if wabs_ptr is not None else None
        sp = timing.span('conv_igemm', cs.flops, cs.abytes)
        stats = want_stats and _BN_EPILOGUE and not relu and cout % 4 == 0
        parts, cap = _stats_request(d, dev) if stats else (None, 0)
        ybits = _amax_zeroed(dev) if (wabs_ptr is not None and not stats) else None
        nparts = _launch_forward(d, x_ptr, xbits, pl_ptr, wabs_ptr, bias, y, 1 if relu else 0, st, parts, cap, ybits, x_pk)
        if ybits is not None:
            _note_amax(y, ybits)
        if nparts > 0:
            bn_parts = (parts, nparts, _PACKED and wabs_ptr is not None and bias is None and cout % 8 == 0
                        and not observers_active() and not _wgrad_planar_pays(d))
    else:
        sp = timing.span('conv_igemm_f32', cs.flops, cs.abytes)
        _C.call('evk_conv2d_fwd', ctypes.byref(d), x_ptr, w_ptr, _ptr(bias), y.data_ptr(), 1 if relu else 0, st)
    timing.stop(sp)
    cs.desc, cs.relu, cs.cin, cs.has_bias, cs.bn_parts = d, relu, cin, bias is not None, bn_parts
    cs.bias_leaf = bias
    cs.w_stride = tuple(weight.stride())
    cs.xk, cs.w_ohwi, cs.y, cs.weight = xk, w_ohwi, (y if relu else None), weight
    return y, cs


def _sparse_dgrad(cs):
    d = cs.desc
    return (_planes_math() and (d.kh < d.stride_h or d.kw < d.stride_w) and d.Cin % 8 == 0 and d.Cout % 8 == 0
            and cs.cin == d.Cin)


def _conv_backward(cs, dy, need_dx, need_dw, need_db, accum=None, inplace=False, accum_bits=None):
    d, dev, st, cin, cout = cs.desc, dy.device, _stream(), cs.cin, cs.desc.Cout
    dy = materialize_lazy(dy)
    if accum_bits is not None and not (need_dx and _f16x2() and d.stride_h == 1 and d.stride_w == 1 and not inplace
                                       and d.Cin == cin and cin % 8 == 0 and cout % 8 == 0):
        accum, accum_bits = materialize_lazy(accum), None
    dy = as_nhwc(dy, 'conv2d.backward')
    dy_pk = _is_packed(dy)
    if dy_pk and (cs.relu or need_db or not _f16x2() or d.Cout % 8 or cs.cin != d.Cin):
        raise HipPathError('conv2d.backward: a packed output gradient reached a convolution that cannot read it')
    if cs.relu:
        g = torch.empty_like(dy)
        _C.call('evk_relu_bwd', dy.data_ptr(), cs.y.data_ptr(), g.data_ptr(), dy.numel(), st)
        dy = g
    x3 = _planes_math()
    cin_p, cout_p, narrow8 = conv_channel_padding(cin, cout, x3)
    dyk = _pad_last(dy.data_ptr(), d.N * d.Ho * d.Wo, cout, cout_p, dev) if cout_p != cout else dy
    dk = _C.ConvDesc(d.N, d.H, d.W, cin_p, d.Ho, d.Wo, cout_p, d.kh, d.kw, d.stride_h, d.stride_w, d.pad_h, d.pad_w,
                     d.dil_h, d.dil_w)
    early = _WGRAD_EARLY_MODE == 1 or (_WGRAD_EARLY_MODE == 2 and need_dw and cout_p == cout and cin_p == cin and not dy_pk
                                       and _wgrad_planar_pays(dk, need_db))
    wgrad_first = early and need_dx and (need_dw or need_db) and _f16x2() and x3
    dx = dw = db = None
    if wgrad_first:
        absmax_bits(dyk, st)
        dw, db = _wgrad(cs, dk, dyk, dy_pk, need_dw, need_db, x3, st)
    if need_dx and x3 and cin_p == cin and (narrow8 or (cout_p == cout and cout % 8 == 0)):
        dx = _dgrad_planes(cs, dk, dyk, dy_pk, narrow8, accum, accum_bits, inplace, st)
    elif need_dx:
        dx = _dgrad_f32(cs, dk, dyk, accum, st)
    if (need_dw or need_db) and not wgrad_first:
        dw, db = _wgrad(cs, dk, dyk, dy_pk, need_dw, need_db, x3, st)
    return dx, dw, db


def _dgrad_planes(cs, dk, dyk, dy_pk, narrow8, accum, accum_bits, inplace, st):
    d, w_ohwi, cin, dev = cs.desc, cs.w_ohwi, cs.cin, dyk.device
    w_src = w_ohwi
    if narrow8:
        taps = d.kh * d.kw
        w_src = torch.zeros((dk.Cout, taps, cin), device=dev, dtype=torch.float32)
        w_src[:d.Cout].copy_(w_ohwi.permute(0, 2, 3, 1).reshape(d.Cout, taps, cin))
    pl_ptr, wabs_ptr, _keep = _weight_planes(cs.weight, w_src, w_src.data_ptr(), dk, 1, st, dev)
    if accum is not None:
        accum = as_nhwc(accum, 'conv2d.backward.accum')
    acc_ptr = _ptr(accum)
    dx = accum if (inplace and accum is not None) else empty_nhwc(d.N, cin, d.H, d.W, dev)
    dybits = absmax_bits(dyk, st) if wabs_ptr is not None else None
    sp = timing.span('conv_igemm', cs.flops, cs.abytes, cs.scope)
    if wabs_ptr is not None:
        hit = getattr(dx, '_evk_amax', None) if inplace else None
        dxbits = hit[2] if hit is not None else _amax_zeroed(dev)
        if accum_bits is not None and acc_ptr is not None:
            relu_bits_stats['masked_dgrad'] += 1
            _C.call('evk_conv2d_dgrad_f16x2_masked', ctypes.byref(dk), dyk.data_ptr(), dybits.data_ptr(), pl_ptr, wabs_ptr,
                    acc_ptr, accum_bits.data_ptr(), dx.data_ptr(), _ptr(dxbits), 4 if dy_pk else 0, st)
        else:
            _C.call('evk_conv2d_dgrad_f16x2_ex', ctypes.byref(dk), dyk.data_ptr(), dybits.data_ptr(), pl_ptr, wabs_ptr, acc_ptr,
                    dx.data_ptr(), _ptr(dxbits), 4 if dy_pk else 0, st)
        if dxbits is not None:
            _note_amax(dx, dxbits)
    else:
        _C.call(_entry('evk_conv2d_dgrad_x3'), ctypes.byref(dk), dyk.data_ptr(), pl_ptr, acc_ptr, dx.data_ptr(), st)
    timing.stop(sp)
    return dx


def _dgrad_f32(cs, dk, dyk, accum, st):
    d, w_ohwi, cin, cout = cs.desc, cs.w_ohwi, cs.cin, cs.desc.Cout
    cin_p, cout_p, taps, dev = dk.Cin, dk.Cout, d.kh * d.kw, w_ohwi.device
    w_src = w_ohwi
    if cin_p != cin or cout_p != cout:
        w_src = torch.zeros((cout_p, taps, cin_p), device=dev, dtype=torch.float32)
        tmp = (_pad_last(w_ohwi.data_ptr(), cout * taps, cin, cin_p, dev) if cin_p != cin
               else w_ohwi.permute(0, 2, 3, 1))
        w_src[:cout].copy_(tmp.reshape(cout, taps, cin_p))
    wt = torch.empty((cin_p, taps, cout_p), device=dev, dtype=torch.float32)
    _C.call('evk_conv2d_pack_dgrad_weight', ctypes.byref(dk), w_src.data_ptr(), wt.data_ptr(), st)
    if accum is not None:
        if cin_p != cin:
            raise HipPathError('conv2d.backward: accum with channel-padded inputs is not supported')
        accum = as_nhwc(accum, 'conv2d.backward.accum')
    dxk = empty_nhwc(d.N, cin_p, d.H, d.W, dev)
    sp = timing.span('conv_igemm_f32', cs.flops, cs.abytes, cs.scope)
    _C.call('evk_conv2d_dgrad', ctypes.byref(dk), dyk.data_ptr(), wt.data_ptr(), _ptr(accum), dxk.data_ptr(), st)
    timing.stop(sp)
    if cin_p == cin:
        return dxk
    dx = empty_nhwc(d.N, cin, d.H, d.W, dev)
    _C.call('evk_unpad_channels', dxk.data_ptr(), dx.data_ptr(), d.N * d.H * d.W, cin_p, cin, st)
    return dx


def _as_param_strides(dw, w_stride, admits):
    if dw.shape[2] * dw.shape[3] == 1 and dw.stride() != w_stride and admits:
        return dw.as_strided(dw.shape, w_stride)
    return dw


def _launch_wgrad(d, x_ptr, dy_ptr, dw, db, ws, ws_bytes, st, x3=True, scales=None, flags=None):
    if scales is not None and flags is not None:
        _C.call('evk_conv2d_wgrad_f16x2_ex', ctypes.byref(d), x_ptr, scales[0].data_ptr(), dy_ptr, scales[1].data_ptr(),
                dw.data_ptr(), _ptr(db), ws.data_ptr(), ws_bytes, flags, st)
    elif scales is not None:
        _C.call('evk_conv2d_wgrad_f16x2', ctypes.byref(d), x_ptr, scales[0].data_ptr(), dy_ptr, scales[1].data_ptr(),
                dw.data_ptr(), _ptr(db), ws.data_ptr(), ws_bytes, st)
    else:
        _C.call(_entry('evk_conv2d_wgrad_x3') if x3 else 'evk_conv2d_wgrad', ctypes.byref(d), x_ptr, dy_ptr, dw.data_ptr(),
                _ptr(db), ws.data_ptr(), ws_bytes, st)


def _wgrad_f16x2_operands(cs, dk, xk, dyk, xbits, dybits, x_pk, dy_pk, need_db, st):
    same_cout = dk.Cout == cs.desc.Cout
    if same_cout and dk.Cin == cs.cin and not x_pk and not dy_pk and _wgrad_planar_pays(dk, need_db):
        xw, dyw = _pack_pass('evk_pack_planar_f16x2', xk, xbits, st), _pack_pass('evk_pack_planar_f16x2', dyk, dybits, st)
        return xw.data_ptr(), dyw.data_ptr(), 8 | 16, (xw, dyw)
    xw, dyw = xk, dyk
    if _PACKED and not need_db and same_cout and _wgrad_pack_pays(cs.flops, 0 if x_pk else xk.numel(),
                                                                  0 if dy_pk else dyk.numel()):
        if not x_pk:
            xw, x_pk = _pack_pass('evk_pack_f16x2', xk, xbits, st), True
        if not dy_pk:
            dyw, dy_pk = _pack_pass('evk_pack_f16x2', dyk, dybits, st), True
    return xw.data_ptr(), dyw.data_ptr(), (2 if x_pk else 0) | (4 if dy_pk else 0), (xw, dyw)


def _pack_pass(entry, t, bits, st):
    out = torch.empty_like(t)
    _C.call(entry, t.data_ptr(), t.numel(), bits.data_ptr(), out.data_ptr(), st)
    return out


def _wgrad(cs, dk, dyk, dy_pk, need_dw, need_db, x3, st):
    d, xk, dev = cs.desc, cs.xk, dyk.device
    cin, cout, cin_p, cout_p, kh, kw, taps = cs.cin, d.Cout, dk.Cin, dk.Cout, d.kh, d.kw, d.kh * d.kw
    lib = _C.load()
    ws_bytes = (lib.evk_conv2d_wgrad_x3_workspace_bytes if x3 else lib.evk_conv2d_wgrad_workspace_bytes)(ctypes.byref(dk))
    dwk = torch.empty((cout_p, taps, cin_p), device=dev, dtype=torch.float32)
    dbk = torch.empty((cout_p,), device=dev, dtype=torch.float32) if need_db else None
    wstr = cs.w_stride
    contract = tuple(wstr) == (taps * cin, 1, kw * cin, cin) or (taps == 1 and wstr[0] == cin and wstr[1] == 1)
    side = _wgrad_side_stream(dev, cs.weight, cs.bias_leaf if need_db else None) if contract else None
    h2 = x3 and _f16x2()
    pre = (absmax_bits(xk, st), absmax_bits(dyk, st), _is_packed(xk)) if (side is not None and _WGRAD_BATCH[0] > 1 and h2) else None
    shared = _WGRAD_SHARED if (_WGRAD_STREAM[0] and _WGRAD_SHARED_ON[0]) else 0
    dw2 = torch.empty((cout_p * taps, cin), device=dev, dtype=torch.float32) if (need_dw and cin_p != cin) else None
    dw = None
    if need_dw:
        dwv = dw2.reshape(cout_p, taps, cin) if dw2 is not None else dwk
        dw = _as_param_strides(dwv[:cout].reshape(cout, kh, kw, cin).permute(0, 3, 1, 2), wstr, wstr[0] == cin and wstr[1] == 1)
    db = dbk[:cout] if need_db else None

    def launch(st):
        ws = workspace(dev, ws_bytes)
        sp = timing.span('conv_wgrad' if x3 else 'conv_wgrad_f32', cs.flops, cs.abytes, cs.scope)
# ... 402 lines not shown
```

ever_amd/hip/pointwise.py:

```python
import ctypes
import os

import torch
from torch.autograd import Function
from torch.autograd.function import once_differentiable

from .. import _C
from . import timing, weight_planes
from .workspace import workspace
from ._base import (
    HipPathError, _AMAX_HANDOFF, _affine_grads, _amax_zeroed, _conv_out, _dx_scale, _hand_scale, _inherit_amax, _note_amax, _ptr,
    _require_cuda, _same_shape_fake, _stream, _take_handoff, _take_parts, _timed_call, as_nhwc, empty_nhwc,
)
from .streams import (
    _note_param_use,
)
from .conv import (
    _weight_ohwi,
)


class _ReluFn(Function):
    @staticmethod
    def forward(ctx, x):
# ... 107 lines not shown


class _Subsample2Fn(Function):
    @staticmethod
    def forward(ctx, x):
        n, c, h, w = x.shape
        y = empty_nhwc(n, c, (h - 1) // 2 + 1, (w - 1) // 2 + 1, x.device)
        _C.call('evk_subsample2_fwd', x.data_ptr(), y.data_ptr(), n, h, w, c, _stream())
        _inherit_amax(y, x)
        ctx.shape = (n, c, h, w)
        return y

    @staticmethod
    @once_differentiable
    def backward(ctx, g):
        n, c, h, w = ctx.shape
        g = as_nhwc(g, 'subsample2.backward')
        dx = empty_nhwc(n, c, h, w, g.device)
        _C.call('evk_subsample2_bwd', g.data_ptr(), dx.data_ptr(), n, h, w, c, _stream())
        return dx


def max_pool1x1s2(x):
    _require_cuda(x, 'max_pool1x1s2')
    x = as_nhwc(x, 'max_pool1x1s2')
    if x.shape[1] % 4:
        raise HipPathError('max_pool1x1s2: channels must be a multiple of 4')
    return _Subsample2Fn.apply(x)


class _BilinearFn(Function):
    @staticmethod
    def forward(ctx, x, ho, wo):
        n, c, h, w = x.shape
        y = empty_nhwc(n, c, ho, wo, x.device)
        _timed_call('resample_loss', 4.0 * (x.numel() + y.numel()), 'evk_upsample_bilinear_fwd', x.data_ptr(),
                    y.data_ptr(), n, h, w, ho, wo, c, _stream())
        ctx.dims = (n, c, h, w, ho, wo)
        return y

    @staticmethod
    @once_differentiable
    def backward(ctx, dy):
        n, c, h, w, ho, wo = ctx.dims
        dy = as_nhwc(dy, 'bilinear.backward')
        dx = empty_nhwc(n, c, h, w, dy.device)
        _timed_call('resample_loss', 4.0 * (dy.numel() + dx.numel()), 'evk_upsample_bilinear_bwd', dy.data_ptr(),
                    dx.data_ptr(), n, h, w, ho, wo, c, _stream())
        return dx, None, None


def upsample_bilinear(x, scale_factor):
    _require_cuda(x, 'upsample_bilinear')
    x = as_nhwc(x, 'upsample_bilinear')
    sh, sw = (scale_factor, scale_factor) if not isinstance(scale_factor, (tuple, list)) else scale_factor
    ho, wo = int(x.shape[2] * sh), int(x.shape[3] * sw)
    return _inherit_amax(_BilinearFn.apply(x, ho, wo), x)


class _GapFn(Function):
    @staticmethod
    def forward(ctx, x):
        n, c, h, w = x.shape
        y = empty_nhwc(n, c, 1, 1, x.device)
        _C.call('evk_gap_fwd', x.data_ptr(), y.data_ptr(), n, h * w, c, _stream())
        ctx.shape = (n, c, h, w)
        return y

    @staticmethod
    @once_differentiable
    def backward(ctx, dy):
        n, c, h, w = ctx.shape
        dy = dy.reshape(n, c).contiguous()
        dx = empty_nhwc(n, c, h, w, dy.device)
        _C.call('evk_gap_bwd', dy.data_ptr(), dx.data_ptr(), n, h * w, c, _stream())
        return dx


def global_avg_pool(x):
    _require_cuda(x, 'global_avg_pool')
    x = as_nhwc(x, 'global_avg_pool')
    return _GapFn.apply(x)


class _RelationFn(Function):
    @staticmethod
    def forward(ctx, scene, content, feat):
        n, c, h, w = content.shape
        out = empty_nhwc(n, c, h, w, content.device)
        r = torch.empty((n, h * w), device=content.device, dtype=torch.float32)
        _C.call('evk_relation_fwd', scene.data_ptr(), content.data_ptr(), feat.data_ptr(), out.data_ptr(),
                r.data_ptr(), n, h * w, c, _stream())
        ctx.save_for_backward(scene, content, feat, r)
        return out

    @staticmethod
    @once_differentiable
    def backward(ctx, dout):
        scene, content, feat, r = ctx.saved_tensors
        n, c, h, w = content.shape
        dev = content.device
        dout = as_nhwc(dout, 'fs_relation.backward')
        lib = _C.load()
        ws_bytes = lib.evk_relation_workspace_bytes(n, h * w, c)
        ws = workspace(dev, ws_bytes)
        dscene = empty_nhwc(n, c, 1, 1, dev)
        dcontent = torch.empty_like(content)
        dfeat = torch.empty_like(feat)
        _C.call('evk_relation_bwd', dout.data_ptr(), scene.data_ptr(), content.data_ptr(), feat.data_ptr(),
                r.data_ptr(), dscene.data_ptr(), dcontent.data_ptr(), dfeat.data_ptr(), n, h * w, c, ws.data_ptr(),
                ws_bytes, _stream())
        return dscene, dcontent, dfeat


def fs_relation(scene, content, feat):
    _require_cuda(content, 'fs_relation')
    content, feat = as_nhwc(content, 'fs_relation.content'), as_nhwc(feat, 'fs_relation.feat')
    n, c, h, w = content.shape
    scene = as_nhwc(scene.reshape(n, c, 1, 1), 'fs_relation.scene')
    return _inherit_amax(_RelationFn.apply(scene, content, feat), feat)


class _RelationBnFn(Function):

    @staticmethod
    def forward(ctx, scene, zc, zf, wc, bc, wf, bf, rmc, rvc, rmf, rvf, cfg):
        (parts_c, parts_f, mom_c, eps_c, mom_f, eps_f) = cfg
        n, c, h, w = zc.shape
        rows, dev, st = n * h * w, zc.device, _stream()
        stats = torch.empty((2, 4, c), device=dev, dtype=torch.float32)
        for k, (parts, g, b, rm, rv, mom, eps) in enumerate(((parts_c, wc, bc, rmc, rvc, mom_c, eps_c),
                                                               (parts_f, wf, bf, rmf, rvf, mom_f, eps_f))):
            _C.call('evk_bn_finalize_parts', parts[0].data_ptr(), parts[1], c, rows, _ptr(g), _ptr(b), _ptr(rm), _ptr(rv),
                    float(mom), float(eps), stats[k, 0].data_ptr(), stats[k, 1].data_ptr(), stats[k, 2].data_ptr(), st)
        out = empty_nhwc(n, c, h, w, dev)
        r = torch.empty((n, h * w), device=dev, dtype=torch.float32)
        abits = _amax_zeroed(dev)
        _C.call('evk_relation_bn_fwd', scene.data_ptr(), zc.data_ptr(), stats[0, 2].data_ptr(), zf.data_ptr(),
                stats[1, 2].data_ptr(), out.data_ptr(), r.data_ptr(), n, h * w, c, _ptr(abits), st)
        _AMAX_HANDOFF[0] = (abits, False)
        ctx.pack = (bool(len(parts_c) > 2 and parts_c[2]), bool(len(parts_f) > 2 and parts_f[2]))
        ctx.save_for_backward(scene, zc, zf, wc, wf, stats, r)
        ctx.mark_non_differentiable(*[t for t in (rmc, rvc, rmf, rvf) if t is not None])
        return out

    @staticmethod
    @once_differentiable
    def backward(ctx, dout):
        scene, zc, zf, wc, wf, stats, r = ctx.saved_tensors
        n, c, h, w = zc.shape
        rows, dev, st = n * h * w, zc.device, _stream()
        dout = as_nhwc(dout, 'fs_relation.backward')
        lib = _C.load()
        nb = int(lib.evk_relation_bn_parts(n, h * w))
        ws_bytes = lib.evk_relation_bn_workspace_bytes(n, h * w, c)
        ws = torch.empty((ws_bytes // 4,), device=dev, dtype=torch.float32)
        dscene = empty_nhwc(n, c, 1, 1, dev)
        gc, gf = torch.empty_like(zc), torch.empty_like(zf)
        _C.call('evk_relation_bn_bwd', dout.data_ptr(), scene.data_ptr(), zc.data_ptr(), stats[0, 2].data_ptr(),
                stats[0, 0].data_ptr(), zf.data_ptr(), stats[1, 2].data_ptr(), stats[1, 0].data_ptr(), r.data_ptr(),
                dscene.data_ptr(), gc.data_ptr(), gf.data_ptr(), n, h * w, c, ws.data_ptr(), ws_bytes, st)
        coef = workspace(dev, 16 * c * 4)
        grads = []
        for k, (g, z, gamma) in enumerate(((gc, zc, wc), (gf, zf, wf))):
            sums = ws[nb * c * (1 + 4 * k):]
            maxima = ws[nb * c * (3 + 4 * k):]
            abits, pack = _dx_scale(dev, ctx.pack[k])
            dz = torch.empty_like(z)
            dgamma, dbeta = _affine_grads(gamma, c, dev)
            _timed_call('bn', 12.0 * z.numel(), 'evk_bn_bwd_from_partials', g.data_ptr(), z.data_ptr(), _ptr(gamma),
                        stats[k, 0].data_ptr(), stats[k, 1].data_ptr(), sums.data_ptr(), maxima.data_ptr(), nb, dz.data_ptr(),
                        _ptr(dgamma), _ptr(dbeta), rows, c, 2 if pack else 0, 1, coef.data_ptr(), 16 * c * 4, _ptr(abits), st)
            grads.append((_hand_scale(dz, abits, pack), dgamma, dbeta))
        (dzc, dgc, dbc), (dzf, dgf, dbf) = grads
        return dscene, dzc, dzf, dgc, dbc, dgf, dbf, None, None, None, None, None


def fs_relation_bn(scene, zc, zf, bn_c, bn_f):
    pc, pf = getattr(zc, '_evk_bn_parts', None), getattr(zf, '_evk_bn_parts', None)
    if pc is None or pf is None or pc[1] <= 0 or pf[1] <= 0 or zc.shape != zf.shape or zc.shape[1] % 4 or zc.shape[1] > 448:
        return None
    _take_parts(zc)
    _take_parts(zf)
    n, c, h, w = zc.shape
    scene = as_nhwc(scene.reshape(n, c, 1, 1), 'fs_relation.scene')
    weight_planes.note_running_stats_changed()
    _AMAX_HANDOFF[0] = None

    def stat(bn, name):
        return getattr(bn, name) if bn.track_running_stats else None
    out = _RelationBnFn.apply(scene, zc, zf, bn_c.weight, bn_c.bias, bn_f.weight, bn_f.bias, stat(bn_c, 'running_mean'),
                              stat(bn_c, 'running_var'), stat(bn_f, 'running_mean'), stat(bn_f, 'running_var'),
                              (pc, pf, bn_c.momentum, bn_c.eps, bn_f.momentum, bn_f.eps))
    return _take_handoff(out)


class _BnReluDotFn(Function):

    @staticmethod
    def forward(ctx, z, gamma, beta, w, bias, rm, rv, cfg):
        parts, mom, eps = cfg
        n, c, h, wd = z.shape
        k = w.shape[0]
        rows, dev, st = n * h * wd, z.device, _stream()
        stats = torch.empty((4, c), device=dev, dtype=torch.float32)
        _C.call('evk_bn_finalize_parts', parts[0].data_ptr(), parts[1], c, rows, _ptr(gamma), _ptr(beta), _ptr(rm), _ptr(rv),
                float(mom), float(eps), stats[0].data_ptr(), stats[1].data_ptr(), stats[2].data_ptr(), st)
        w2 = _weight_ohwi(w.detach()).reshape(k, c)
        out = empty_nhwc(n, k, h, wd, dev)
        _timed_call('bn', 4.0 * z.numel(), 'evk_bn_relu_dot_fwd', z.data_ptr(), stats[2].data_ptr(), w2.data_ptr(), _ptr(bias),
                    out.data_ptr(), rows, c, k, st)
        ctx.pack = bool(len(parts) > 2 and parts[2])
        ctx.has_bias = bias is not None
        ctx.save_for_backward(z, gamma, w, stats)
        ctx.mark_non_differentiable(*[t for t in (rm, rv) if t is not None])
        return out

    @staticmethod
    @once_differentiable
    def backward(ctx, dl):
        z, gamma, w, stats = ctx.saved_tensors
        n, c, h, wd = z.shape
        k = w.shape[0]
        rows, dev, st = n * h * wd, z.device, _stream()
        dl = as_nhwc(dl, 'bn_relu_dot.backward')
        lib = _C.load()
        ws_bytes = lib.evk_bn_relu_dot_workspace_bytes(rows, c, k)
        ws = workspace(dev, ws_bytes)
        abits, pack = _dx_scale(dev, ctx.pack)
        dz = torch.empty_like(z)
        dgamma, dbeta = _affine_grads(gamma, c, dev)
        dw = torch.empty_strided(w.shape, w.stride(), device=dev, dtype=torch.float32) if (
            w.stride(0) == c and w.stride(1) == 1) else torch.empty_like(w, memory_format=torch.channels_last)
        dbias = torch.empty((k,), device=dev, dtype=torch.float32) if ctx.has_bias else None
        w2 = _weight_ohwi(w.detach()).reshape(k, c)
        _timed_call('bn', 12.0 * z.numel(), 'evk_bn_relu_dot_bwd', dl.data_ptr(), z.data_ptr(), stats[2].data_ptr(), _ptr(gamma),
                    stats[0].data_ptr(), stats[1].data_ptr(), w2.data_ptr(), dz.data_ptr(), _ptr(dgamma), _ptr(dbeta),
                    dw.data_ptr(), _ptr(dbias), rows, c, k, 2 if pack else 0, ws.data_ptr(), ws_bytes, _ptr(abits), st)
        return _hand_scale(dz, abits, pack), dgamma, dbeta, dw, dbias, None, None, None


def bn_relu_dot_admits(c, k, kernel_shape=(1, 1)):
    return (tuple(kernel_shape) == (1, 1) and 1 <= k <= 16 and c > 0 and c % 4 == 0 and c <= 1024
            and (c <= 256 or k <= 4) and 16 * (4 + k) * c <= 65536)


def bn_relu_dot(z, bn, conv):
    parts = getattr(z, '_evk_bn_parts', None)
    k, c = conv.weight.shape[0], z.shape[1]
    if (parts is None or parts[1] <= 0 or conv.weight.shape[1] != c
            or not bn_relu_dot_admits(c, k, conv.weight.shape[2:])):
        return None
    _take_parts(z)
    weight_planes.note_running_stats_changed()
    if torch.is_grad_enabled():
        _note_param_use(conv.weight, conv.bias)
    rm = bn.running_mean if bn.track_running_stats else None
    rv = bn.running_var if bn.track_running_stats else None
    return _BnReluDotFn.apply(z, bn.weight, bn.bias, conv.weight, conv.bias, rm, rv, (parts, bn.momentum, bn.eps))


class _Mean4Fn(Function):
    @staticmethod
    def forward(ctx, a, b, c, d):
        out = torch.empty_like(a)
        bits = _amax_zeroed(a.device)
        _C.call('evk_mean4_fwd', a.data_ptr(), b.data_ptr(), c.data_ptr(), d.data_ptr(), out.data_ptr(), a.numel(),
                _ptr(bits), _stream())
        if bits is not None:
            _note_amax(out, bits)
        return out

    @staticmethod
    @once_differentiable
    def backward(ctx, g):
        g = as_nhwc(g, 'mean4.backward')
        q = torch.empty_like(g)
        _C.call('evk_scale', g.data_ptr(), 0.25, q.data_ptr(), g.numel(), _stream())
        return q, q, q, q


def mean4(a, b, c, d):
    ts = [as_nhwc(t, 'mean4') for t in (a, b, c, d)]
    for t in ts[1:]:
        if t.shape != ts[0].shape:
            raise ValueError('mean4: shape mismatch')
    return _Mean4Fn.apply(*ts)


from . import oplib as _oplib


_relu_plain, _add_plain, _max_pool_plain, _nearest_add_plain = relu, add, max_pool3x3s2, upsample_nearest2x_add
_bilinear_plain, _gap_plain, _relation_plain, _mean4_plain = upsample_bilinear, global_avg_pool, fs_relation, mean4
relu = _oplib.traceable('relu', '(Tensor x) -> Tensor', _relu_plain, adapt=lambda x: (x,), fake=_same_shape_fake)
add = _oplib.traceable('add', '(Tensor a, Tensor b) -> Tensor', _add_plain, adapt=lambda a, b: (a, b), fake=_same_shape_fake)
max_pool3x3s2 = _oplib.traceable(
    'max_pool3x3s2', '(Tensor x) -> Tensor', _max_pool_plain, adapt=lambda x: (x,),
    fake=lambda x: _oplib.nhwc_like(x, x.shape[0], x.shape[1], _conv_out(x.shape[2], 3, 2, 1, 1), _conv_out(x.shape[3], 3, 2, 1, 1)))
upsample_nearest2x_add = _oplib.traceable(
    'upsample_nearest2x_add', '(Tensor top, Tensor lateral) -> Tensor', _nearest_add_plain, adapt=lambda top, lateral: (top, lateral),
    fake=lambda top, lateral: _oplib.nhwc_like(lateral, *lateral.shape))
upsample_bilinear = _oplib.traceable(
    'upsample_bilinear', '(Tensor x, float scale_h, float scale_w) -> Tensor',
    _bilinear_plain, impl_fn=lambda x, sh, sw: _bilinear_plain(x, (sh, sw)),
    adapt=lambda x, scale_factor: (x,) + tuple(float(s) for s in ((scale_factor, scale_factor) if not isinstance(
        scale_factor, (tuple, list)) else scale_factor)),
    fake=lambda x, sh, sw: _oplib.nhwc_like(x, x.shape[0], x.shape[1], int(x.shape[2] * sh), int(x.shape[3] * sw)))
global_avg_pool = _oplib.traceable('global_avg_pool', '(Tensor x) -> Tensor', _gap_plain, adapt=lambda x: (x,),
                                   fake=lambda x: _oplib.nhwc_like(x, x.shape[0], x.shape[1], 1, 1))
fs_relation = _oplib.traceable('fs_relation', '(Tensor scene, Tensor content, Tensor feat) -> Tensor', _relation_plain,
                               adapt=lambda scene, content, feat: (scene, content, feat),
                               fake=lambda scene, content, feat: _oplib.nhwc_like(feat, *feat.shape))
mean4 = _oplib.traceable('mean4', '(Tensor a, Tensor b, Tensor c, Tensor d) -> Tensor', _mean4_plain,
                         adapt=lambda a, b, c, d: (a, b, c, d), fake=lambda a, b, c, d: _oplib.nhwc_like(a, *a.shape))
```

include/ever_hip.h:

```cpp
#ifndef EVER_HIP_H_
#define EVER_HIP_H_

#include <stddef.h>
#include <stdint.h>

#ifdef __cplusplus
extern "C" {
#endif

#define EVK_OK 0
#define EVK_E_INVALID (-1)
#define EVK_E_UNSUPPORTED (-2)
#define EVK_E_LAUNCH (-3)
#define EVK_E_WORKSPACE (-4)

const char* evk_last_error(void);
int evk_abi_version(void);
const char* evk_build_arch(void);

typedef struct evk_conv_desc {
  int32_t N, H, W, Cin;
  int32_t Ho, Wo, Cout;
  int32_t kh, kw;
  int32_t stride_h, stride_w;
// ... 199 lines not shown
                               int32_t C, void* stream);

int evk_subsample2_fwd(const float* x, float* y, int32_t N, int32_t H, int32_t W, int32_t C, void* stream);
int evk_subsample2_bwd(const float* dy, float* dx, int32_t N, int32_t H, int32_t W, int32_t C, void* stream);

int evk_upsample_bilinear_fwd(const float* x, float* y, int32_t N, int32_t Hi, int32_t Wi,
                              int32_t Ho, int32_t Wo, int32_t C, void* stream);
int evk_upsample_bilinear_bwd(const float* dy, float* dx, int32_t N, int32_t Hi, int32_t Wi,
                              int32_t Ho, int32_t Wo, int32_t C, void* stream);
int evk_upsample_bilinear_plan(int32_t N, int32_t Hi, int32_t Wi, int32_t Ho, int32_t Wo, int32_t C, int32_t vec,
                               int32_t backward, int32_t* out);
int evk_upsample_bilinear_slice_fwd(const float* x, float* y, int32_t N, int32_t Hi, int32_t Wi, int32_t Ho,
                                    int32_t Wo, int32_t C, int32_t c0, int32_t Ctot, void* stream);
int evk_upsample_bilinear_slice_bwd(const float* dy, float* dx, int32_t N, int32_t Hi, int32_t Wi, int32_t Ho,
                                    int32_t Wo, int32_t C, int32_t c0, int32_t Ctot, void* stream);

int evk_hr_fuse_fwd(const float* const* terms, const int32_t* shifts, const float* const* scale_shifts, int32_t nterms,
                    float* y, uint32_t* relu_bits, uint32_t* y_absmax, int32_t N, int32_t H, int32_t W, int32_t C,
                    void* stream);
int evk_hr_fuse_bwd(const float* dy, const uint32_t* relu_bits, float* dmasked, float* dpooled1, float* dpooled2,
                    float* dpooled3, int32_t N, int32_t H, int32_t W, int32_t C, void* stream);

int evk_wfuse_fwd(const float* const* terms, const int32_t* shifts, int32_t nterms, const float* weights, int32_t norm,
                  float eps, float* y, int32_t N, int32_t H, int32_t W, int32_t C, void* stream);
int evk_wfuse_bwd(const float* dy, const float* const* terms, const int32_t* shifts, int32_t nterms, const float* weights,
                  int32_t norm, float eps, float* const* dterms, float* dweights, void* workspace, int64_t workspace_bytes,
                  int32_t N, int32_t H, int32_t W, int32_t C, void* stream);
size_t evk_wfuse_workspace_bytes(int32_t N, int32_t H, int32_t W, int32_t C, int32_t nterms);
int evk_wfuse_plan(int32_t N, int32_t H, int32_t W, int32_t C, int32_t nterms, int32_t* out);

int evk_d4_apply(const float* x, float* y, int32_t N, int32_t Hi, int32_t Wi, int32_t C, int32_t op, void* stream);
int evk_d4_merge(const float* const* terms, const int32_t* ops, int32_t nterms, const float* acc, float* y, int32_t N,
                 int32_t Ho, int32_t Wo, int32_t C, int32_t count, void* stream);
int evk_d4_plan(int32_t N, int32_t Hi, int32_t Wi, int32_t C, int32_t op, int32_t* out);
int evk_d4_force_kernel(int32_t kernel);

int evk_augment_batch(const int64_t* records, const int64_t* table, int32_t N, int32_t C, int32_t crop_h, int32_t crop_w,
                      int32_t Ho, int32_t Wo, const float* mean, const float* std, int32_t mask_pad_value, int32_t nchw,
                      int32_t src_f32, int32_t mask_mode, float* out, void* out_mask, void* stream);
int evk_augment_plan(int32_t Hs, int32_t Ws, int32_t C, int32_t op, int32_t y0, int32_t x0, int32_t crop_h, int32_t crop_w,
                     int32_t Ho, int32_t Wo, int32_t src_f32, int32_t nchw, int32_t* out);
int evk_augment_force_kernel(int32_t kernel);

int evk_gap_fwd(const float* x, float* y, int32_t N, int32_t HW, int32_t C, void* stream);
int evk_gap_bwd(const float* dy, float* dx, int32_t N, int32_t HW, int32_t C, void* stream);

int evk_relation_fwd(const float* scene, const float* content, const float* feat, float* out,
                     float* r, int32_t N, int32_t HW, int32_t C, void* stream);
size_t evk_relation_workspace_bytes(int32_t N, int32_t HW, int32_t C);
int evk_relation_bwd(const float* dout, const float* scene, const float* content, const float* feat,
                     const float* r, float* dscene, float* dcontent, float* dfeat, int32_t N,
                     int32_t HW, int32_t C, void* workspace, size_t workspace_bytes, void* stream);

int evk_mean4_fwd(const float* a, const float* b, const float* c, const float* d, float* out,
                  int64_t n, uint32_t* out_absmax, void* stream);

int64_t evk_loss_stats_doubles(int32_t K);

int evk_bce_fwd(const float* logits, const int64_t* labels, int64_t npix, int64_t ignore_index,
                float label_smoothing, float* loss, double* stats, void* stream);
int evk_bce_bwd(const float* logits, const int64_t* labels, int64_t npix, int64_t ignore_index,
                float label_smoothing, const double* stats, const float* grad_scale, float* dlogits,
                int32_t accumulate, void* stream);

int evk_bce_fwd_ex(const float* logits, const int64_t* labels, int64_t npix, int64_t ignore_index,
                   float label_smoothing, float pos_weight, int32_t reduction, float* loss, double* stats, void* stream);
int evk_bce_bwd_ex(const float* logits, const int64_t* labels, int64_t npix, int64_t ignore_index,
                   float label_smoothing, float pos_weight, int32_t reduction, const double* stats,
                   const float* grad_scale, float* dlogits, int32_t accumulate, void* stream);

int evk_dice_stats(const float* logits, const int64_t* labels, int64_t npix, int32_t C,
                   int64_t ignore_index, double* stats, void* stream);
int evk_dice_finish(const double* stats, int32_t C, float smooth, int32_t ignore_channel,
                    float* loss, void* stream);
int evk_dice_bwd(const float* logits, const int64_t* labels, int64_t npix, int32_t C,
                 int64_t ignore_index, const double* stats, float smooth, int32_t ignore_channel,
                 const float* grad_scale, float* dlogits, int32_t accumulate, void* stream);

int evk_ce_fwd(const float* logits, const int64_t* labels, int64_t npix, int32_t C,
               int64_t ignore_index, float label_smoothing, float* loss, double* stats, void* stream);
int evk_ce_bwd(const float* logits, const int64_t* labels, int64_t npix, int32_t C,
               int64_t ignore_index, float label_smoothing, const double* stats,
               const float* grad_scale, float* dlogits, int32_t accumulate, void* stream);

int evk_soft_ce_fwd(const float* logits, const float* target, int64_t npix, int32_t C, float* loss,
                    double* stats, void* stream);
int evk_soft_ce_bwd(const float* logits, const float* target, int64_t npix, int32_t C,
                    const float* grad_scale, float* dlogits, void* stream);

int32_t evk_opt_blocks_per_tensor(void);
int evk_sqnorm_multi(const float* const* grads, const int64_t* sizes, int32_t ntensors,
                     double* partial, float max_norm, float* total_norm, float* clip_coef,
                     void* stream);
int evk_sgd_multi(float* const* params, const float* const* grads, float* const* momentum_bufs,
                  const int64_t* sizes, int32_t ntensors, float lr, float momentum, float dampening,
                  float weight_decay, int32_t nesterov, int32_t first_step,
                  const float* clip_coef , void* stream);
int evk_sgd_multi_lr(float* const* params, const float* const* grads, float* const* momentum_bufs,
                     const int64_t* sizes, int32_t ntensors, float lr, const float* lr_dev, float momentum,
                     float dampening, float weight_decay, int32_t nesterov, int32_t first_step,
                     const float* clip_coef, void* stream);
int evk_adam_multi(float* const* params, const float* const* grads, float* const* exp_avg, float* const* exp_avg_sq,
                   const int64_t* sizes, int32_t ntensors, float lr, float beta1, float beta2, float eps,
                   float weight_decay, int32_t decoupled, float bias_correction1, float sqrt_bias_correction2,
                   const float* clip_coef , void* stream);

int64_t evk_prob_stats_doubles(int32_t C);
int evk_prob_stats(const float* logits, const int64_t* labels, int64_t npix, int32_t C,
                   int64_t ignore_index, double* stats, void* stream);
int evk_prob_stats_bwd(const float* logits, const int64_t* labels, int64_t npix, int32_t C,
                       int64_t ignore_index, const float* g_tp, const float* g_sp, float* dlogits,
                       int32_t accumulate, void* stream);
int evk_focal_fwd(const float* logits, const float* target, int64_t n, float gamma, float alpha,
                  int32_t mode, int32_t mean, float* loss, double* stats, void* stream);
int evk_focal_bwd(const float* logits, const float* target, int64_t n, float gamma, float alpha,
                  int32_t mode, int32_t mean, const float* grad_scale, float* dlogits, void* stream);
int evk_confusion_matrix(const int64_t* y_true, const int64_t* y_pred, int64_t n, int32_t num_classes,
                         int64_t* cm, void* stream);
int evk_confusion_from_logits(const float* logits, const int64_t* y_true, int64_t npix,
                              int32_t C_logits, int32_t num_classes, int64_t* cm, void* stream);

size_t evk_gn_workspace_bytes(int32_t N, int64_t HW, int32_t C, int32_t G);
int evk_gn_plan(int64_t HW, int32_t C, int32_t* out);
int evk_gn_fwd(const float* x, const float* gamma, const float* beta, float eps, float* y,
               float* save_mean, float* save_rstd, int32_t N, int64_t HW, int32_t C, int32_t G,
               uint32_t flags, void* workspace, size_t workspace_bytes, void* stream);
int evk_gn_bwd(const float* dy, const float* x, const float* y, const float* gamma,
               const float* save_mean, const float* save_rstd, float* dx, float* dgamma, float* dbeta,
               int32_t N, int64_t HW, int32_t C, int32_t G, uint32_t flags, void* workspace,
               size_t workspace_bytes, void* stream);
int evk_concat_channels(const float* a, const float* b, float* out, int64_t rows, int32_t Ca,
                        int32_t Cb, void* stream);
int evk_split_channels(const float* src, float* a, float* b, int64_t rows, int32_t Ca, int32_t Cb,
                       void* stream);
int evk_channel_scale(const float* x, const float* scale, float* y, int32_t N, int64_t HW, int32_t C,
                      void* stream);

int evk_bn_finalize_parts(const float* parts, int32_t nparts, int32_t C, int64_t rows, const float* gamma, const float* beta,
                          float* running_mean, float* running_var, float momentum, float eps, float* save_mean,
                          float* save_invstd, float* scale_shift, void* stream);
int evk_relation_bn_fwd(const float* scene, const float* zc, const float* scale_shift_c, const float* zf,
                        const float* scale_shift_f, float* out, float* r, int32_t N, int32_t HW, int32_t C,
                        uint32_t* out_absmax, void* stream);
int32_t evk_relation_bn_parts(int32_t N, int32_t HW);
size_t evk_relation_bn_workspace_bytes(int32_t N, int32_t HW, int32_t C);
int evk_relation_bn_bwd(const float* dout, const float* scene, const float* zc, const float* scale_shift_c,
                        const float* mean_invstd_c, const float* zf, const float* scale_shift_f, const float* mean_invstd_f,
                        const float* r, float* dscene, float* gc, float* gf, int32_t N, int32_t HW, int32_t C, void* workspace,
                        size_t workspace_bytes, void* stream);
int evk_bn_bwd_from_partials(const float* g, const float* x, const float* gamma, const float* save_mean,
                             const float* save_invstd, const float* partial, const float* maxima, int32_t nparts, float* dx,
                             float* dgamma, float* dbeta, int64_t rows, int32_t C, uint32_t flags, int32_t train,
                             void* workspace, size_t workspace_bytes, uint32_t* dx_absmax, void* stream);

int evk_bn_relu_dot_plan(int64_t rows, int32_t C, int32_t K, int32_t* out);
int evk_bn_relu_dot_fwd(const float* z, const float* scale_shift, const float* w, const float* bias, float* out, int64_t rows,
                        int32_t C, int32_t K, void* stream);
size_t evk_bn_relu_dot_workspace_bytes(int64_t rows, int32_t C, int32_t K);
int evk_bn_relu_dot_bwd(const float* dl, const float* z, const float* scale_shift, const float* gamma, const float* save_mean,
                        const float* save_invstd, const float* w, float* dz, float* dgamma, float* dbeta, float* dw,
                        float* dbias, int64_t rows, int32_t C, int32_t K, uint32_t flags, void* workspace,
                        size_t workspace_bytes, uint32_t* dx_absmax, void* stream);

int evk_bn_local_stats(const float* x, double* stats, int64_t rows, int32_t C, void* workspace,
                       size_t workspace_bytes, void* stream);
int evk_bn_apply_stats(const float* x, const float* residual, const float* gamma, const float* beta,
                       const float* mean, const float* invstd, float* y, int64_t rows, int32_t C,
                       uint32_t flags, void* workspace, size_t workspace_bytes, void* stream);
int evk_bn_bwd_local_sums(const float* dy, const float* x, const float* y, const float* gamma,
                          const float* beta, const float* mean, const float* invstd, float* d_residual,
                          double* sums, int64_t rows, int32_t C, uint32_t flags, void* workspace,
                          size_t workspace_bytes, void* stream);
int evk_bn_bwd_apply_sums(const float* dy, const float* x, const float* y, const float* gamma,
                          const float* beta, const float* mean, const float* invstd, const float* mean_g,
                          const float* mean_gx, float* dx, int64_t rows, int32_t C, uint32_t flags,
                          void* workspace, size_t workspace_bytes, void* stream);

int evk_pack_multi(const float* const* srcs, const int64_t* sizes, const int64_t* offsets,
                   int32_t ntensors, float scale, float* dst, void* stream);

int evk_ce_pixel_fwd(const float* logits, const int64_t* labels, int64_t npix, int32_t C,
                     int64_t ignore_index, float* loss_pix, void* stream);
int evk_ce_pixel_bwd(const float* logits, const int64_t* labels, int64_t npix, int32_t C,
                     int64_t ignore_index, const float* grad_pix, float* dlogits, void* stream);
int64_t evk_ohem_state_bytes(void);
int evk_ohem_fwd(const float* losses, int64_t n, int64_t keep, float* loss, void* state, void* stream);
int evk_ohem_bwd(const float* losses, int64_t n, void* state, const float* grad_scale, float* dlosses,
                 void* stream);

int evk_depthwise_fwd(const evk_conv_desc* d, const float* x, const float* w, const float* bias, float* y,
                      uint32_t flags, void* stream);
size_t evk_depthwise_bwd_workspace_bytes(const evk_conv_desc* d);
int evk_depthwise_bwd(const evk_conv_desc* d, const float* dy, const float* x, const float* y, const float* w,
                      float* dx, float* dw, float* db, void* workspace, size_t workspace_bytes, void* stream);
int evk_broadcast_hw(const float* src, float* dst, int32_t N, int64_t HW, int32_t C, void* stream);
int evk_sum_hw(const float* src, float* dst, int32_t N, int64_t HW, int32_t C, void* stream);

int evk_ln_plan(int64_t R, int32_t C, int32_t* out );
size_t evk_ln_bwd_workspace_bytes(int64_t R, int32_t C);
int evk_ln_fwd(const float* x, const float* gamma, const float* beta, float eps, float* y, float* save_mean,
               float* save_rstd, int64_t R, int32_t C, void* stream);
int evk_ln_bwd(const float* dy, const float* x, const float* save_mean, const float* save_rstd, const float* gamma,
               float* dx, float* dgamma, float* dbeta, int64_t R, int32_t C, void* workspace, size_t workspace_bytes,
               void* stream);
int evk_scale_residual_fwd(const float* a, const float* z, const float* gamma, const float* sample_scale, float* y,
                           int32_t N, int64_t HW, int32_t C, void* stream);
size_t evk_scale_residual_bwd_workspace_bytes(int32_t N, int64_t HW, int32_t C);
int evk_scale_residual_bwd(const float* dy, const float* z, const float* gamma, const float* sample_scale, float* dz,
                           float* dgamma, int32_t N, int64_t HW, int32_t C, void* workspace, size_t workspace_bytes,
                           void* stream);

#ifdef __cplusplus
}
#endif
#endif
```

Baseline: 565.9 tiles/s.

## Recompute relation gradients in a second pass to fuse BN dx and conv bias grad

Result: no change. 570.9 tiles/s, median of 4 (+0.9%).

```diff
diff --git a/ever_amd/_C.py b/ever_amd/_C.py
--- a/ever_amd/_C.py
+++ b/ever_amd/_C.py
@@ -104,6 +104,9 @@
     'evk_relation_bn_workspace_bytes': (c_size_t, [c_i32, c_i32, c_i32]),
     'evk_relation_bn_bwd': (c_int, [P, P, P, P, P, P, P, P, P, P, P, P, c_i32, c_i32, c_i32, P, c_size_t, P]),
     'evk_bn_bwd_from_partials': (c_int, [P, P, P, P, P, P, P, c_i32, P, P, P, c_i64, c_i32, c_u32, c_i32, P, c_size_t, P, P]),
+    'evk_relation_bn_dz_workspace_bytes': (c_size_t, [c_i32, c_i32, c_i32]),
+    'evk_relation_bn_bwd_sums': (c_int, [P, P, P, P, P, P, P, P, P, P, c_i32, c_i32, c_i32, P, c_size_t, P]),
+    'evk_relation_bn_bwd_dz': (c_int, [P] * 18 + [c_i32, c_i32, c_i32, P, c_size_t, P, P, P]),
     'evk_bn_bwd_bits': (c_int, [P, P, P, P, P, P, P, P, P, P, P, c_i64, c_i32, c_u32, c_i32, P, c_size_t, P, P, P]),
     'evk_bn_fwd_train_parts_dual': (c_int, [P, P, P, P, P, P, c_f32, c_f32, P, P, P, P, c_f32, c_f32, P, P, P, P, P, c_i64, c_i32,
                                             P, c_i32, P, c_i32, P, c_size_t, P, P, P]),
diff --git a/ever_amd/csrc/bn.hip b/ever_amd/csrc/bn.hip
--- a/ever_amd/csrc/bn.hip
+++ b/ever_amd/csrc/bn.hip
@@ -288,13 +288,6 @@
     if (bits) atomicMax(&amax[0], bits);
   }
 }
-struct BnBwdFinalSet {
-  const float *partial, *gamma, *invstd;
-  float *dgamma, *dbeta, *coef;
-  int train;
-  uint32_t* amax;
-  const float* pmax;
-};
 template <typename Set, int NR>
 struct BnFinalSets {
   Set row[NR];
@@ -310,27 +303,6 @@
   bn_bwd_final_body<kFinCh>(s.partial, nblk, C, inv_rows, s.gamma, s.invstd, s.dgamma, s.dbeta, s.coef, s.train, s.amax, s.pmax);
 }
 
-struct BnDxCoef {
-  f32x4 k0, k1, k2, mu, is;
-};
-__device__ __forceinline__ BnDxCoef bn_dx_coef(const float* __restrict__ coef, const float* __restrict__ mean,
-                                               const float* __restrict__ invstd, int C, int c) {
-  return {reinterpret_cast<const f32x4*>(coef)[c], reinterpret_cast<const f32x4*>(coef + C)[c],
-          reinterpret_cast<const f32x4*>(coef + 2 * C)[c], reinterpret_cast<const f32x4*>(mean)[c],
-          reinterpret_cast<const f32x4*>(invstd)[c]};
-}
-template <bool PK>
-__device__ __forceinline__ f32x4 bn_dx_store(const BnDxCoef& k, const f32x4 g, const f32x4 xv, float* __restrict__ dx, size_t i,
-                                             float pk_inv) {
-  const f32x4 xh = (xv - k.mu) * k.is;
-  const f32x4 out = k.k0 * (g - k.k1 - xh * k.k2);
-  if constexpr (PK) {
-    reinterpret_cast<u32x4*>(dx)[i] = pack_hl4(out, pk_inv);
-  } else {
-    reinterpret_cast<f32x4*>(dx)[i] = out;
-  }
-  return out;
-}
 template <bool PK>
 __global__ __launch_bounds__(256) void bn_bwd_apply_kernel(const float* __restrict__ dy, const float* __restrict__ x,
                                                            const float* __restrict__ y, const float* __restrict__ mean,
@@ -484,8 +456,7 @@
   launch_parts_final_sets(st, s, nullptr, C, rows);
 }
 
-static void launch_bn_bwd_final_sets(hipStream_t st, const BnBwdFinalSet& a, const BnBwdFinalSet* b, int nblk, int C,
-                                     int64_t rows) {
+void launch_bn_bwd_final_sets(hipStream_t st, const BnBwdFinalSet& a, const BnBwdFinalSet* b, int nblk, int C, int64_t rows) {
   const dim3 grid((C + kFinCh - 1) / kFinCh, b ? 2 : 1);
   const double inv_rows = 1.0 / (double)rows;
   if (b) hipLaunchKernelGGL(bn_bwd_final_kernel<2>, grid, dim3(256), 0, st, BnFinalSets<BnBwdFinalSet, 2>{{a, *b}}, nblk, C, inv_rows);
diff --git a/ever_amd/csrc/bn_common.hpp b/ever_amd/csrc/bn_common.hpp
--- a/ever_amd/csrc/bn_common.hpp
+++ b/ever_amd/csrc/bn_common.hpp
@@ -178,11 +178,42 @@
   }
 }
 
+struct BnDxCoef {
+  f32x4 k0, k1, k2, mu, is;
+};
+__device__ __forceinline__ BnDxCoef bn_dx_coef(const float* __restrict__ coef, const float* __restrict__ mean,
+                                               const float* __restrict__ invstd, int C, int c) {
+  return {reinterpret_cast<const f32x4*>(coef)[c], reinterpret_cast<const f32x4*>(coef + C)[c],
+          reinterpret_cast<const f32x4*>(coef + 2 * C)[c], reinterpret_cast<const f32x4*>(mean)[c],
+          reinterpret_cast<const f32x4*>(invstd)[c]};
+}
+template <bool PK>
+__device__ __forceinline__ f32x4 bn_dx_store(const BnDxCoef& k, const f32x4 g, const f32x4 xv, float* __restrict__ dx, size_t i,
+                                             float pk_inv) {
+  const f32x4 xh = (xv - k.mu) * k.is;
+  const f32x4 out = k.k0 * (g - k.k1 - xh * k.k2);
+  if constexpr (PK) {
+    reinterpret_cast<u32x4*>(dx)[i] = pack_hl4(out, pk_inv);
+  } else {
+    reinterpret_cast<f32x4*>(dx)[i] = out;
+  }
+  return out;
+}
+
+struct BnBwdFinalSet {
+  const float *partial, *gamma, *invstd;
+  float *dgamma, *dbeta, *coef;
+  int train;
+  uint32_t* amax;
+  const float* pmax;
+};
+
 void launch_parts_final(hipStream_t st, const float* parts, int nparts, int C, double rows, const float* gamma,
                         const float* beta, float* running_mean, float* running_var, float momentum, float eps,
                         float* save_mean, float* save_invstd, float* scale_shift, uint32_t* amax, int pack);
 void launch_bn_bwd_final(hipStream_t st, const float* partial, int nblk, int C, int64_t rows, const float* gamma,
                          const float* invstd, float* dgamma, float* dbeta, float* coef, int train, uint32_t* amax,
                          const float* pmax);
-
-}
+void launch_bn_bwd_final_sets(hipStream_t st, const BnBwdFinalSet& a, const BnBwdFinalSet* b, int nblk, int C, int64_t rows);
+
+}
diff --git a/ever_amd/csrc/conv_wgrad.hip b/ever_amd/csrc/conv_wgrad.hip
--- a/ever_amd/csrc/conv_wgrad.hip
+++ b/ever_amd/csrc/conv_wgrad.hip
@@ -140,7 +140,10 @@
   hipLaunchKernelGGL(colsum_partial_kernel, dim3(nblk), dim3(256), 0, st, src, workspace, rows, c, rpb);
   int rc = check_launch("colsum_partial");
   if (rc) return rc;
-  hipLaunchKernelGGL(colsum_final_kernel, dim3((c + 7) / 8), dim3(256), 0, st, (const float*)workspace, out, nblk, c);
+  return launch_colsum_final(workspace, out, nblk, c, st);
+}
+int launch_colsum_final(const float* partial, float* out, int nblk, int c, hipStream_t st) {
+  hipLaunchKernelGGL(colsum_final_kernel, dim3((c + 7) / 8), dim3(256), 0, st, partial, out, nblk, c);
   return check_launch("colsum_final");
 }
 
diff --git a/ever_amd/csrc/relation.hip b/ever_amd/csrc/relation.hip
--- a/ever_amd/csrc/relation.hip
+++ b/ever_amd/csrc/relation.hip
@@ -1,9 +1,12 @@
 #include "stream_common.hpp"
+#include "bn_common.hpp"
+#include "wgrad_common.hpp"
 
 namespace evk {
 
 __device__ __forceinline__ f32x4 bn_relu4(const f32x4 z, const f32x4 sc, const f32x4 sh) {
-  f32x4 y = z * sc + sh;
+  f32x4 y = {__builtin_fmaf(z.x, sc.x, sh.x), __builtin_fmaf(z.y, sc.y, sh.y), __builtin_fmaf(z.z, sc.z, sh.z),
+             __builtin_fmaf(z.w, sc.w, sh.w)};
   y.x = fmaxf(y.x, 0.f); y.y = fmaxf(y.y, 0.f); y.z = fmaxf(y.z, 0.f); y.w = fmaxf(y.w, 0.f);
   return y;
 }
@@ -107,7 +110,47 @@
   }
 }
 
+__device__ __forceinline__ float relation_dot4(const f32x4 a, const f32x4 y) {
+  float t;
+  {
+#pragma clang fp contract(off)
+    t = a.y * y.y;
+  }
+  return __builtin_fmaf(a.w, y.w, __builtin_fmaf(a.z, y.z, __builtin_fmaf(a.x, y.x, t)));
+}
 template <int NCH>
+__device__ __forceinline__ float relation_bn_pixel(const f32x4 (&a)[NCH], const f32x4 (&zfv)[NCH], const f32x4 (&zcv)[NCH],
+                                                   const f32x4 (&s4)[NCH], const f32x4 (&scc)[NCH], const f32x4 (&shc)[NCH],
+                                                   const f32x4 (&scf)[NCH], const f32x4 (&shf)[NCH], const float rv,
+                                                   f32x4 (&yc)[NCH], f32x4 (&gc)[NCH], f32x4 (&gf)[NCH]) {
+  float dot = 0.f;
+#pragma unroll
+  for (int j = 0; j < NCH; ++j) {
+    const f32x4 y = bn_relu4(zfv[j], scf[j], shf[j]);
+    f32x4 g;
+    {
+#pragma clang fp contract(off)
+      dot = dot + relation_dot4(a[j], y);
+      g = a[j] * rv;
+    }
+    gf[j] = relu_mask(g, y);
+  }
+  dot = wave_sum(dot);
+  const float dz = dot * rv * (1.f - rv);
+#pragma unroll
+  for (int j = 0; j < NCH; ++j) {
+    yc[j] = bn_relu4(zcv[j], scc[j], shc[j]);
+    f32x4 g;
+    {
+#pragma clang fp contract(off)
+      g = s4[j] * dz;
+    }
+    gc[j] = relu_mask(g, yc[j]);
+  }
+  return dz;
+}
+
+template <int NCH, bool STORE_G>
 __global__ __launch_bounds__(256) void relation_bn_bwd_kernel(
     const float* __restrict__ dout, const float* __restrict__ scene, const float* __restrict__ zc,
     const float* __restrict__ ssc, const float* __restrict__ mic, const float* __restrict__ zf, const float* __restrict__ ssf,
@@ -139,9 +182,6 @@
     muf[j] = ok ? *reinterpret_cast<const f32x4*>(mif + cb * 4) : zero4;
     isf[j] = ok ? *reinterpret_cast<const f32x4*>(mif + C + cb * 4) : zero4;
   }
-  auto amax4 = [](f32x4& m, const f32x4 v) {
-    m.x = fmaxf(m.x, fabsf(v.x)); m.y = fmaxf(m.y, fabsf(v.y)); m.z = fmaxf(m.z, fabsf(v.z)); m.w = fmaxf(m.w, fabsf(v.w));
-  };
   for (int p = p0 + wave; p < p1; p += 4) {
     const size_t pix = (size_t)n * HW + p;
     const float rv = r[pix];
@@ -154,36 +194,26 @@
       zfv[j] = ok ? *reinterpret_cast<const f32x4*>(zf + pix * C + cb * 4) : zero4;
       zcv[j] = ok ? *reinterpret_cast<const f32x4*>(zc + pix * C + cb * 4) : zero4;
     }
-    float dot = 0.f;
+    f32x4 yc[NCH], gcv[NCH], gfv[NCH];
+    const float dz = relation_bn_pixel<NCH>(a, zfv, zcv, s4, scc, shc, scf, shf, rv, yc, gcv, gfv);
 #pragma unroll
     for (int j = 0; j < NCH; ++j) {
       const int cb = lane + 64 * j;
-      const f32x4 y = bn_relu4(zfv[j], scf[j], shf[j]);
-      dot += a[j].x * y.x + a[j].y * y.y + a[j].z * y.z + a[j].w * y.w;
-      f32x4 g = a[j] * rv;
-      g.x = y.x > 0.f ? g.x : 0.f; g.y = y.y > 0.f ? g.y : 0.f; g.z = y.z > 0.f ? g.z : 0.f; g.w = y.w > 0.f ? g.w : 0.f;
-      if (cb < c4) *reinterpret_cast<f32x4*>(gf + pix * C + cb * 4) = g;
-      const f32x4 xh = (zfv[j] - muf[j]) * isf[j];
-      acc[j][5] += g;
-      acc[j][6] += g * xh;
-      amax4(acc[j][7], g);
-      amax4(acc[j][8], xh);
-    }
-    dot = wave_sum(dot);
-    const float dz = dot * rv * (1.f - rv);
-#pragma unroll
-    for (int j = 0; j < NCH; ++j) {
-      const int cb = lane + 64 * j;
-      const f32x4 y = bn_relu4(zcv[j], scc[j], shc[j]);
-      f32x4 g = s4[j] * dz;
-      g.x = y.x > 0.f ? g.x : 0.f; g.y = y.y > 0.f ? g.y : 0.f; g.z = y.z > 0.f ? g.z : 0.f; g.w = y.w > 0.f ? g.w : 0.f;
-      if (cb < c4) *reinterpret_cast<f32x4*>(gc + pix * C + cb * 4) = g;
-      acc[j][0] += y * dz;
-      const f32x4 xh = (zcv[j] - muc[j]) * isc[j];
-      acc[j][1] += g;
-      acc[j][2] += g * xh;
-      amax4(acc[j][3], g);
-      amax4(acc[j][4], xh);
+      if (STORE_G && cb < c4) {
+        *reinterpret_cast<f32x4*>(gf + pix * C + cb * 4) = gfv[j];
+        *reinterpret_cast<f32x4*>(gc + pix * C + cb * 4) = gcv[j];
+      }
+      const f32x4 xhf = (zfv[j] - muf[j]) * isf[j];
+      acc[j][5] += gfv[j];
+      acc[j][6] += gfv[j] * xhf;
+      absmax4(acc[j][7], gfv[j]);
+      absmax4(acc[j][8], xhf);
+      acc[j][0] += yc[j] * dz;
+      const f32x4 xhc = (zcv[j] - muc[j]) * isc[j];
+      acc[j][1] += gcv[j];
+      acc[j][2] += gcv[j] * xhc;
+      absmax4(acc[j][3], gcv[j]);
+      absmax4(acc[j][4], xhc);
     }
   }
   float* my = sacc + (size_t)wave * 9 * C;
@@ -214,6 +244,84 @@
   }
 }
 
+template <int NCH>
+__global__ __launch_bounds__(256) void relation_bn_dz_kernel(
+    const float* __restrict__ dout, const float* __restrict__ scene, const float* __restrict__ zc,
+    const float* __restrict__ ssc, const float* __restrict__ mic, const float* __restrict__ coef_c,
+    const float* __restrict__ zf, const float* __restrict__ ssf, const float* __restrict__ mif,
+    const float* __restrict__ coef_f, const float* __restrict__ r, float* __restrict__ dzc, float* __restrict__ dzf,
+    float* __restrict__ colpart, uint32_t* __restrict__ amax_c, uint32_t* __restrict__ amax_f, int HW, int C, int pix_per_blk,
+    int nblk) {
+  extern __shared__ __attribute__((aligned(16))) float sacc[];
+  const int c4 = C >> 2;
+  const int lane = threadIdx.x & 63, wave = threadIdx.x >> 6;
+  const int bx = (int)bn_blk(), n = (int)(gridDim.y - 1u - blockIdx.y);
+  const int p0 = bx * pix_per_blk, p1 = min(HW, p0 + pix_per_blk);
+  const float* sc = scene + (size_t)n * C;
+  const f32x4 zero4 = {0.f, 0.f, 0.f, 0.f};
+  const BnDxCoef kzero = {zero4, zero4, zero4, zero4, zero4};
+  f32x4 s4[NCH], scc[NCH], shc[NCH], scf[NCH], shf[NCH], sum_c[NCH], sum_f[NCH];
+  BnDxCoef kc[NCH], kf[NCH];
+#pragma unroll
+  for (int j = 0; j < NCH; ++j) {
+    const int cb = lane + 64 * j;
+    const bool ok = cb < c4;
+    sum_c[j] = sum_f[j] = zero4;
+    s4[j] = ok ? *reinterpret_cast<const f32x4*>(sc + cb * 4) : zero4;
+    scc[j] = ok ? *reinterpret_cast<const f32x4*>(ssc + cb * 4) : zero4;
+    shc[j] = ok ? *reinterpret_cast<const f32x4*>(ssc + C + cb * 4) : zero4;
+    scf[j] = ok ? *reinterpret_cast<const f32x4*>(ssf + cb * 4) : zero4;
+    shf[j] = ok ? *reinterpret_cast<const f32x4*>(ssf + C + cb * 4) : zero4;
+    kc[j] = ok ? bn_dx_coef(coef_c, mic, mic + C, C, cb) : kzero;
+    kf[j] = ok ? bn_dx_coef(coef_f, mif, mif + C, C, cb) : kzero;
+  }
+  uint32_t mc = 0, mf = 0;
+  for (int p = p0 + wave; p < p1; p += 4) {
+    const size_t pix = (size_t)n * HW + p;
+    const size_t e0 = pix * c4;
+    const float rv = r[pix];
+    f32x4 a[NCH], zfv[NCH], zcv[NCH];
+#pragma unroll
+    for (int j = 0; j < NCH; ++j) {
+      const int cb = lane + 64 * j;
+      const bool ok = cb < c4;
+      a[j] = ok ? bn_ld(dout, e0 + cb) : zero4;
+      zfv[j] = ok ? bn_ld(zf, e0 + cb) : zero4;
+      zcv[j] = ok ? bn_ld(zc, e0 + cb) : zero4;
+    }
+    f32x4 yc[NCH], gcv[NCH], gfv[NCH];
+    relation_bn_pixel<NCH>(a, zfv, zcv, s4, scc, shc, scf, shf, rv, yc, gcv, gfv);
+#pragma unroll
+    for (int j = 0; j < NCH; ++j) {
+      const int cb = lane + 64 * j;
+      if (cb < c4) {
+        const f32x4 of = bn_dx_store<false>(kf[j], gfv[j], zfv[j], dzf, e0 + cb, 1.f);
+        const f32x4 oc = bn_dx_store<false>(kc[j], gcv[j], zcv[j], dzc, e0 + cb, 1.f);
+        sum_f[j] += of;
+        sum_c[j] += oc;
+        mf = abs4_bits(mf, of);
+        mc = abs4_bits(mc, oc);
+      }
+    }
+  }
+  if (amax_c) commit_absmax(amax_c, mc > 0x7f800000u ? 0x7fc00000u : mc);
+  if (amax_f) commit_absmax(amax_f, mf > 0x7f800000u ? 0x7fc00000u : mf);
+  float* my = sacc + (size_t)wave * 2 * C;
+#pragma unroll
+  for (int j = 0; j < NCH; ++j) {
+    const int cb = lane + 64 * j;
+    if (cb < c4) {
+      *reinterpret_cast<f32x4*>(my + cb * 4) = sum_c[j];
+      *reinterpret_cast<f32x4*>(my + C + cb * 4) = sum_f[j];
+    }
+  }
+  __syncthreads();
+  const size_t blk = (size_t)n * nblk + bx;
+  const int W2 = 2 * C;
+  for (int c = threadIdx.x; c < W2; c += 256)
+    colpart[blk * W2 + c] = (sacc[c] + sacc[W2 + c]) + (sacc[2 * W2 + c] + sacc[3 * W2 + c]);
+}
+
 static int relation_blocks(int HW) {
   constexpr int ppb = 64, cap = 256;
   int b = (HW + ppb - 1) / ppb;
@@ -256,6 +364,30 @@
 extern "C" int32_t evk_relation_bn_parts(int32_t N, int32_t HW) { return (int32_t)relation_records(N, HW); }
 extern "C" size_t evk_relation_bn_workspace_bytes(int32_t N, int32_t HW, int32_t C) {
   return C > 0 ? relation_records(N, HW) * C * 9 * sizeof(float) : 0;
+}
+static int relation_bn_bwd_pass1(const char* what, const float* dout, const float* scene, const float* zc,
+                                 const float* scale_shift_c, const float* mean_invstd_c, const float* zf,
+                                 const float* scale_shift_f, const float* mean_invstd_f, const float* r, float* dscene, float* gc,
+                                 float* gf, int N, int HW, int C, void* workspace, hipStream_t st) {
+  const size_t nb = relation_records(N, HW);
+  float* w = (float*)workspace;
+  float* partial = w;
+  float* bnp_c = w + nb * C;
+  float* bnm_c = w + nb * 3 * C;
+  float* bnp_f = w + nb * 5 * C;
+  float* bnm_f = w + nb * 7 * C;
+  const size_t lds = (size_t)4 * 9 * C * sizeof(float);
+  EVK_REQUIRE(lds <= 64 * 1024, EVK_E_UNSUPPORTED, "%s: C=%d does not fit the LDS", what, C);
+  return relation_bwd_launch(what, partial, dscene, N, HW, C, st, [&](int nblk, int ppb) {
+    auto launch = [&](auto kernel) {
+      hipLaunchKernelGGL(kernel, dim3(nblk, N), dim3(256), lds, st, dout, scene, zc, scale_shift_c, mean_invstd_c, zf,
+                         scale_shift_f, mean_invstd_f, r, gc, gf, partial, bnp_c, bnm_c, bnp_f, bnm_f, HW, C, ppb, nblk);
+      return 0;
+    };
+    pick<1, 2, 4>((C / 4 + 63) / 64, [&](auto NCH) {
+      return gc ? launch(relation_bn_bwd_kernel<NCH(), true>) : launch(relation_bn_bwd_kernel<NCH(), false>);
+    });
+  });
 }
 extern "C" int evk_relation_bn_bwd(const float* dout, const float* scene, const float* zc, const float* scale_shift_c,
                                    const float* mean_invstd_c, const float* zf, const float* scale_shift_f,
@@ -268,24 +400,61 @@
   EVK_REQUIRE(nhwc4_ok(N, HW, 1, C) && C <= 448, EVK_E_UNSUPPORTED, "relation_bn_bwd: C=%d", C);
   EVK_REQUIRE(workspace && workspace_bytes >= evk_relation_bn_workspace_bytes(N, HW, C), EVK_E_WORKSPACE,
               "relation_bn_bwd: workspace too small");
+  return relation_bn_bwd_pass1("relation_bn_bwd", dout, scene, zc, scale_shift_c, mean_invstd_c, zf, scale_shift_f,
+                               mean_invstd_f, r, dscene, gc, gf, N, HW, C, workspace, (hipStream_t)stream);
+}
+
+extern "C" size_t evk_relation_bn_dz_workspace_bytes(int32_t N, int32_t HW, int32_t C) {
+  return C > 0 && relation_records(N, HW) ? (relation_records(N, HW) * 11 + 8) * C * sizeof(float) : 0;
+}
+extern "C" int evk_relation_bn_bwd_sums(const float* dout, const float* scene, const float* zc, const float* scale_shift_c,
+                                        const float* mean_invstd_c, const float* zf, const float* scale_shift_f,
+                                        const float* mean_invstd_f, const float* r, float* dscene, int32_t N, int32_t HW,
+                                        int32_t C, void* workspace, size_t workspace_bytes, void* stream) {
+  EVK_REQUIRE(dout && scene && zc && scale_shift_c && mean_invstd_c && zf && scale_shift_f && mean_invstd_f && r && dscene,
+              EVK_E_INVALID, "relation_bn_bwd_sums: null pointer");
+  EVK_REQUIRE(nhwc4_ok(N, HW, 1, C) && C <= 448, EVK_E_UNSUPPORTED, "relation_bn_bwd_sums: C=%d", C);
+  EVK_REQUIRE(workspace && workspace_bytes >= evk_relation_bn_dz_workspace_bytes(N, HW, C), EVK_E_WORKSPACE,
+              "relation_bn_bwd_sums: workspace too small");
+  return relation_bn_bwd_pass1("relation_bn_bwd_sums", dout, scene, zc, scale_shift_c, mean_invstd_c, zf, scale_shift_f,
+                               mean_invstd_f, r, dscene, nullptr, nullptr, N, HW, C, workspace, (hipStream_t)stream);
+}
+extern "C" int evk_relation_bn_bwd_dz(const float* dout, const float* scene, const float* zc, const float* scale_shift_c,
+                                      const float* mean_invstd_c, const float* gamma_c, const float* zf,
+                                      const float* scale_shift_f, const float* mean_invstd_f, const float* gamma_f,
+                                      const float* r, float* dzc, float* dzf, float* dgamma_c, float* dbeta_c, float* dgamma_f,
+                                      float* dbeta_f, float* dbias, int32_t N, int32_t HW, int32_t C, void* workspace,
+                                      size_t workspace_bytes, uint32_t* dzc_absmax, uint32_t* dzf_absmax, void* stream) {
+  EVK_REQUIRE(dout && scene && zc && scale_shift_c && mean_invstd_c && zf && scale_shift_f && mean_invstd_f && r && dzc && dzf &&
+                  dbias,
+              EVK_E_INVALID, "relation_bn_bwd_dz: null pointer");
+  EVK_REQUIRE(nhwc4_ok(N, HW, 1, C) && C <= 448, EVK_E_UNSUPPORTED, "relation_bn_bwd_dz: C=%d", C);
+  EVK_REQUIRE(workspace && workspace_bytes >= evk_relation_bn_dz_workspace_bytes(N, HW, C), EVK_E_WORKSPACE,
+              "relation_bn_bwd_dz: workspace too small");
+  hipStream_t st = (hipStream_t)stream;
   const size_t nb = relation_records(N, HW);
   float* w = (float*)workspace;
-  float* partial = w;
-  float* bnp_c = w + nb * C;
-  float* bnm_c = w + nb * 3 * C;
-  float* bnp_f = w + nb * 5 * C;
-  float* bnm_f = w + nb * 7 * C;
-  hipStream_t st = (hipStream_t)stream;
-  const size_t lds = (size_t)4 * 9 * C * sizeof(float);
-  EVK_REQUIRE(lds <= 64 * 1024, EVK_E_UNSUPPORTED, "relation_bn_bwd: C=%d does not fit the LDS", C);
-  return relation_bwd_launch("relation_bn_bwd", partial, dscene, N, HW, C, st, [&](int nblk, int ppb) {
-    pick<1, 2, 4>((C / 4 + 63) / 64, [&](auto NCH) {
-      hipLaunchKernelGGL(relation_bn_bwd_kernel<NCH()>, dim3(nblk, N), dim3(256), lds, st, dout, scene, zc, scale_shift_c,
-                         mean_invstd_c, zf, scale_shift_f, mean_invstd_f, r, gc, gf, partial, bnp_c, bnm_c, bnp_f, bnm_f, HW, C,
-                         ppb, nblk);
-      return 0;
-    });
+  float* colpart = w + nb * 9 * C;
+  float* coef_c = w + nb * 11 * C;
+  float* coef_f = coef_c + 4 * (size_t)C;
+  const int64_t rows = (int64_t)N * HW;
+  const BnBwdFinalSet fc = {w + nb * C, gamma_c, mean_invstd_c + C, dgamma_c, dbeta_c, coef_c, 1, dzc_absmax, nullptr};
+  const BnBwdFinalSet ff = {w + nb * 5 * C, gamma_f, mean_invstd_f + C, dgamma_f, dbeta_f, coef_f, 1, dzf_absmax, nullptr};
+  launch_bn_bwd_final_sets(st, fc, &ff, (int)nb, C, rows);
+  int rc = check_launch("bn_bwd_final_dual");
+  if (rc) return rc;
+  const int nblk = relation_blocks(HW);
+  const int ppb = (HW + nblk - 1) / nblk;
+  const size_t lds = (size_t)4 * 2 * C * sizeof(float);
+  pick<1, 2>((C / 4 + 63) / 64, [&](auto NCH) {
+    hipLaunchKernelGGL(relation_bn_dz_kernel<NCH()>, dim3(nblk, N), dim3(256), lds, st, dout, scene, zc, scale_shift_c,
+                       mean_invstd_c, (const float*)coef_c, zf, scale_shift_f, mean_invstd_f, (const float*)coef_f, r, dzc, dzf,
+                       colpart, dzc_absmax, dzf_absmax, HW, C, ppb, nblk);
+    return 0;
   });
+  rc = check_launch("relation_bn_dz");
+  if (rc) return rc;
+  return launch_colsum_final(colpart, dbias, (int)nb, 2 * C, st);
 }
 extern "C" size_t evk_relation_workspace_bytes(int32_t N, int32_t HW, int32_t C) {
   return C > 0 ? relation_records(N, HW) * C * sizeof(float) : 0;
diff --git a/ever_amd/csrc/wgrad_common.hpp b/ever_amd/csrc/wgrad_common.hpp
--- a/ever_amd/csrc/wgrad_common.hpp
+++ b/ever_amd/csrc/wgrad_common.hpp
@@ -51,5 +51,6 @@
 
 size_t colsum_workspace_bytes(int64_t rows, int c);
 int launch_colsum(const float* src, float* out, int64_t rows, int c, float* workspace, hipStream_t st);
+int launch_colsum_final(const float* partial, float* out, int nblk, int c, hipStream_t st);
 
 }
diff --git a/ever_amd/hip/conv.py b/ever_amd/hip/conv.py
--- a/ever_amd/hip/conv.py
+++ b/ever_amd/hip/conv.py
@@ -184,8 +184,19 @@
             and cs.cin == d.Cin)
 
 
+def _handed_bias_grad(dy, cout):
+    hit = getattr(dy, '_evk_bias_grad', None)
+    if hit is None or hit[0] != dy._version or hit[1] != dy.data_ptr() or hit[2].numel() != cout or dy.shape[1] != cout:
+        return None
+    return hit[2]
+
+
 def _conv_backward(cs, dy, need_dx, need_dw, need_db, accum=None, inplace=False, accum_bits=None):
     d, dev, st, cin, cout = cs.desc, dy.device, _stream(), cs.cin, cs.desc.Cout
+    db_in = _handed_bias_grad(dy, cout) if (need_db and not cs.relu) else None
+    if db_in is not None:
+        dx, dw, _ = _conv_backward(cs, dy, need_dx, need_dw, False, accum, inplace, accum_bits)
+        return dx, dw, db_in
     dy = materialize_lazy(dy)
     if accum_bits is not None and not (need_dx and _f16x2() and d.stride_h == 1 and d.stride_w == 1 and not inplace
                                        and d.Cin == cin and cin % 8 == 0 and cout % 8 == 0):
diff --git a/ever_amd/hip/pointwise.py b/ever_amd/hip/pointwise.py
--- a/ever_amd/hip/pointwise.py
+++ b/ever_amd/hip/pointwise.py
@@ -283,6 +283,8 @@
         rows, dev, st = n * h * w, zc.device, _stream()
         dout = as_nhwc(dout, 'fs_relation.backward')
         lib = _C.load()
+        if not any(ctx.pack):
+            return _RelationBnFn._backward_two_pass(dout, scene, zc, zf, wc, wf, stats, r, lib, st)
         nb = int(lib.evk_relation_bn_parts(n, h * w))
         ws_bytes = lib.evk_relation_bn_workspace_bytes(n, h * w, c)
         ws = torch.empty((ws_bytes // 4,), device=dev, dtype=torch.float32)
@@ -304,6 +306,29 @@
                         _ptr(dgamma), _ptr(dbeta), rows, c, 2 if pack else 0, 1, coef.data_ptr(), 16 * c * 4, _ptr(abits), st)
             grads.append((_hand_scale(dz, abits, pack), dgamma, dbeta))
         (dzc, dgc, dbc), (dzf, dgf, dbf) = grads
+        return dscene, dzc, dzf, dgc, dbc, dgf, dbf, None, None, None, None, None
+
+    @staticmethod
+    def _backward_two_pass(dout, scene, zc, zf, wc, wf, stats, r, lib, st):
+        n, c, h, w = zc.shape
+        dev, t = zc.device, float(zc.numel())
+        ws_bytes = lib.evk_relation_bn_dz_workspace_bytes(n, h * w, c)
+        ws = torch.empty((ws_bytes // 4,), device=dev, dtype=torch.float32)
+        dscene = empty_nhwc(n, c, 1, 1, dev)
+        _timed_call('bn', 12.0 * t, 'evk_relation_bn_bwd_sums', dout.data_ptr(), scene.data_ptr(), zc.data_ptr(),
+                    stats[0, 2].data_ptr(), stats[0, 0].data_ptr(), zf.data_ptr(), stats[1, 2].data_ptr(), stats[1, 0].data_ptr(),
+                    r.data_ptr(), dscene.data_ptr(), n, h * w, c, ws.data_ptr(), ws_bytes, st)
+        dzc, dzf = torch.empty_like(zc), torch.empty_like(zf)
+        (abits_c, _), (abits_f, _) = _dx_scale(dev, False), _dx_scale(dev, False)
+        (dgc, dbc), (dgf, dbf) = _affine_grads(wc, c, dev), _affine_grads(wf, c, dev)
+        dbias = torch.empty((2, c), device=dev, dtype=torch.float32)
+        _timed_call('bn', 20.0 * t, 'evk_relation_bn_bwd_dz', dout.data_ptr(), scene.data_ptr(), zc.data_ptr(),
+                    stats[0, 2].data_ptr(), stats[0, 0].data_ptr(), _ptr(wc), zf.data_ptr(), stats[1, 2].data_ptr(),
+                    stats[1, 0].data_ptr(), _ptr(wf), r.data_ptr(), dzc.data_ptr(), dzf.data_ptr(), _ptr(dgc), _ptr(dbc),
+                    _ptr(dgf), _ptr(dbf), dbias.data_ptr(), n, h * w, c, ws.data_ptr(), ws_bytes, _ptr(abits_c), _ptr(abits_f), st)
+        dzc, dzf = _hand_scale(dzc, abits_c, False), _hand_scale(dzf, abits_f, False)
+        for dz, db in ((dzc, dbias[0]), (dzf, dbias[1])):
+            dz._evk_bias_grad = (dz._version, dz.data_ptr(), db)
         return dscene, dzc, dzf, dgc, dbc, dgf, dbf, None, None, None, None, None
 
 
diff --git a/include/ever_hip.h b/include/ever_hip.h
--- a/include/ever_hip.h
+++ b/include/ever_hip.h
@@ -375,6 +375,17 @@
                              const float* save_invstd, const float* partial, const float* maxima, int32_t nparts, float* dx,
                              float* dgamma, float* dbeta, int64_t rows, int32_t C, uint32_t flags, int32_t train,
                              void* workspace, size_t workspace_bytes, uint32_t* dx_absmax, void* stream);
+size_t evk_relation_bn_dz_workspace_bytes(int32_t N, int32_t HW, int32_t C);
+int evk_relation_bn_bwd_sums(const float* dout, const float* scene, const float* zc, const float* scale_shift_c,
+                             const float* mean_invstd_c, const float* zf, const float* scale_shift_f,
+                             const float* mean_invstd_f, const float* r, float* dscene, int32_t N, int32_t HW, int32_t C,
+                             void* workspace, size_t workspace_bytes, void* stream);
+int evk_relation_bn_bwd_dz(const float* dout, const float* scene, const float* zc, const float* scale_shift_c,
+                           const float* mean_invstd_c, const float* gamma_c, const float* zf, const float* scale_shift_f,
+                           const float* mean_invstd_f, const float* gamma_f, const float* r, float* dzc, float* dzf,
+                           float* dgamma_c, float* dbeta_c, float* dgamma_f, float* dbeta_f, float* dbias, int32_t N, int32_t HW,
+                           int32_t C, void* workspace, size_t workspace_bytes, uint32_t* dzc_absmax, uint32_t* dzf_absmax,
+                           void* stream);
 
 int evk_bn_relu_dot_plan(int64_t rows, int32_t C, int32_t K, int32_t* out);
 int evk_bn_relu_dot_fwd(const float* z, const float* scale_shift, const float* w, const float* bias, float* out, int64_t rows,
```
